# SmartBFT-Go/consensus

Hardware: NVIDIA H100
Metric: ECDSA-P256 verifies/sec at batch=64K (higher is better)
Workload: dtype u32 limbs (integer)

## Files before the change

consensus_b200/csrc/engine.cu:

```cuda
#include <cuda_runtime.h>
#include <dlfcn.h>

#include <algorithm>
#include <cstdarg>
#include <cstdio>
#include <cstdlib>
#include <cstring>
#include <mutex>
#include <string>
#include <vector>

#include "engine.h"
#include "sha256.cuh"
#include "quorum.cuh"

using namespace sbv;

namespace {

int env_int(const char *name, int dflt) {
    const char *v = getenv(name);
    return v && *v ? atoi(v) : dflt;
}

size_t fbytes(uint8_t curve) { return curve == SBV_P256 ? 32 : 48; }

bool is_pinned(const void *p) {
    cudaPointerAttributes a;
    if (cudaPointerGetAttributes(&a, p) != cudaSuccess) { cudaGetLastError(); return false; }
    return a.type == cudaMemoryTypeHost;
}

__global__ void k_mad_probe(uint32_t *out, uint32_t iters) {
    uint32_t a = threadIdx.x * 2654435761u + 12345u, b = blockIdx.x * 40503u + 777u;
    uint64_t acc[8];
#pragma unroll
    for (int i = 0; i < 8; i++) acc[i] = a + i;
    for (uint32_t it = 0; it < iters; it++) {
#pragma unroll
        for (int i = 0; i < 8; i++) acc[i] = (uint64_t)a * (uint32_t)(b + i) + acc[i];
        a ^= (uint32_t)acc[3];
    }
    uint64_t s = 0;
#pragma unroll
    for (int i = 0; i < 8; i++) s += acc[i];
    if (s == 0x1234567) out[0] = (uint32_t)s;
}

}

int sbv_ensure_scratch(sbv_engine *e, Dev &d, size_t bytes) {
    if (bytes <= d.scratch_cap) return 0;
    CU(e, cudaSetDevice(d.ordinal));
    if (d.d_scratch) cudaFree(d.d_scratch);
    d.d_scratch = nullptr;
    d.scratch_cap = 0;
    size_t cap = bytes + bytes / 4 + 4096;
    CU(e, cudaMalloc(&d.d_scratch, cap));
    d.scratch_cap = cap;
    return 0;
}

int sbv_lane_acquire(sbv_engine *e) {
    std::unique_lock<std::mutex> lk(e->mu);
    int lane = -1;
    e->lane_cv.wait(lk, [&] {
        for (int i = 0; i < SBV_LANES; i++)
            if (!e->lane_busy[i]) { lane = i; return true; }
        return false;
    });
    e->lane_busy[lane] = true;
    return lane;
}
void sbv_lane_release(sbv_engine *e, int lane) {
    { std::lock_guard<std::mutex> lk(e->mu); e->lane_busy[lane] = false; }
    e->lane_cv.notify_one();
}
int sbv_lane_ensure(sbv_engine *e, Dev &d, Dev::Lane &ln, size_t n, size_t pinned_bytes) {
    if (!ln.stream) CU(e, cudaStreamCreateWithFlags(&ln.stream, cudaStreamNonBlocking));
    if (n > ln.cap) {
        CU(e, cudaStreamSynchronize(ln.stream));
        uint8_t **ptrs[] = {&ln.d_r, &ln.d_s, &ln.d_qx, &ln.d_qy, &ln.d_dig, &ln.d_ok};
        for (auto p : ptrs) { if (*p) cudaFree(*p); *p = nullptr; }
        if (ln.d_slot) cudaFree(ln.d_slot);
        ln.d_slot = nullptr;
        ln.cap = 0;
        const size_t cap = n + n / 8 + 1024;
        CU(e, cudaMalloc(&ln.d_r, cap * 48));
        CU(e, cudaMalloc(&ln.d_s, cap * 48));
        CU(e, cudaMalloc(&ln.d_qx, cap * 48));
        CU(e, cudaMalloc(&ln.d_qy, cap * 48));
        CU(e, cudaMalloc(&ln.d_dig, cap * 64));
        CU(e, cudaMalloc(&ln.d_ok, cap));
        CU(e, cudaMalloc(&ln.d_slot, cap * 4));
        ln.cap = cap;
    }
    if (pinned_bytes > ln.h_pin_cap) {
        CU(e, cudaStreamSynchronize(ln.stream));
        if (ln.h_pin) cudaFreeHost(ln.h_pin);
        ln.h_pin = nullptr;
        ln.h_pin_cap = 0;
        const size_t cap = pinned_bytes + pinned_bytes / 4 + 4096;
        CU(e, cudaHostAlloc(&ln.h_pin, cap, cudaHostAllocPortable));
        ln.h_pin_cap = cap;
    }
    (void)d;
    return 0;
}
int sbv_lane_ensure_msgs(sbv_engine *e, Dev::Lane &ln, size_t bytes, size_t n_off) {
    if (!ln.stream) CU(e, cudaStreamCreateWithFlags(&ln.stream, cudaStreamNonBlocking));
    if (bytes > ln.msg_cap) {
        CU(e, cudaStreamSynchronize(ln.stream));
        if (ln.d_msgs) cudaFree(ln.d_msgs);
        ln.d_msgs = nullptr;
        ln.msg_cap = 0;
        const size_t cap = bytes + bytes / 8 + 4096;
        CU(e, cudaMalloc(&ln.d_msgs, cap));
        ln.msg_cap = cap;
    }
    if (n_off > ln.off_cap) {
        CU(e, cudaStreamSynchronize(ln.stream));
        if (ln.d_off) cudaFree(ln.d_off);
        if (ln.d_perm) cudaFree(ln.d_perm);
        ln.d_off = nullptr;
        ln.d_perm = nullptr;
        ln.off_cap = 0;
        const size_t cap = n_off + n_off / 8 + 1024;
        CU(e, cudaMalloc(&ln.d_off, cap * sizeof(uint64_t)));
        CU(e, cudaMalloc(&ln.d_perm, (cap + 3 * 1024) * sizeof(uint32_t)));
        ln.off_cap = cap;
    }
    return 0;
}
int sbv_lane_ensure_aux(sbv_engine *e, Dev::Lane &ln, size_t bytes) {
    if (!ln.stream) CU(e, cudaStreamCreateWithFlags(&ln.stream, cudaStreamNonBlocking));
    if (bytes <= ln.aux_cap) return 0;
    CU(e, cudaStreamSynchronize(ln.stream));
    if (ln.d_aux) cudaFree(ln.d_aux);
    if (ln.h_aux) cudaFreeHost(ln.h_aux);
    ln.d_aux = nullptr; ln.h_aux = nullptr; ln.aux_cap = 0;
    const size_t cap = bytes + bytes / 4 + 4096;
    CU(e, cudaMalloc(&ln.d_aux, cap));
    CU(e, cudaHostAlloc(&ln.h_aux, cap, cudaHostAllocPortable));
    ln.aux_cap = cap;
    return 0;
}
int sbv_launch_sha256(sbv_engine *e, size_t n, const uint8_t *d_msgs, const uint64_t *d_off, uint64_t base, uint8_t *d_digest, uint32_t *d_perm,
                      cudaStream_t st) {
    const uint32_t *perm = nullptr;
    if (d_perm && n >= 2048) {
        uint32_t *hist = d_perm + n, *start = hist + SHA_BINS, *cursor = start + SHA_BINS;
        CU(e, cudaMemsetAsync(hist, 0, SHA_BINS * sizeof(uint32_t), st));
        k_sha_hist<<<(uint32_t)((n + 255) / 256), 256, 0, st>>>((uint32_t)n, d_off, hist);
        k_sha_scan<<<1, SHA_BINS, 0, st>>>(hist, start, cursor);
        k_sha_scatter<<<(uint32_t)((n + 255) / 256), 256, 0, st>>>((uint32_t)n, d_off, start, cursor, d_perm);
        e->launches += 3;
        perm = d_perm;
    }
    k_sha256<<<(uint32_t)((n + 127) / 128), 128, 0, st>>>((uint32_t)n, d_msgs, d_off, base, d_digest, perm);
    e->launches += 1;
    CU(e, cudaGetLastError());
    return 0;
}
int sbv_lane_h2d(sbv_engine *e, Dev::Lane &ln, void *dst, const void *src, size_t bytes, size_t &stage_off, cudaStream_t st) {
    if (bytes == 0) return 0;
    if (!st) st = ln.stream;
    if (is_pinned(src)) {
        CU(e, cudaMemcpyAsync(dst, src, bytes, cudaMemcpyHostToDevice, st));
    } else {
        if (stage_off + bytes > ln.h_pin_cap) return fail(e, SBV_ERR_NOMEM, "pinned staging area too small (%zu + %zu > %zu)", stage_off, bytes, ln.h_pin_cap);
        memcpy(ln.h_pin + stage_off, src, bytes);
        CU(e, cudaMemcpyAsync(dst, ln.h_pin + stage_off, bytes, cudaMemcpyHostToDevice, st));
        stage_off += (bytes + 255) & ~(size_t)255;
    }
    return 0;
}

namespace {

struct NcclUniqueId { char internal[128]; };
typedef int (*nccl_comm_init_all_t)(void **comms, int ndev, const int *devlist);
typedef int (*nccl_comm_init_rank_t)(void **comm, int nranks, NcclUniqueId id, int rank);
typedef int (*nccl_get_unique_id_t)(NcclUniqueId *id);
typedef int (*nccl_comm_destroy_t)(void *comm);
typedef int (*nccl_group_t)(void);
typedef int (*nccl_all_gather_t)(const void *send, void *recv, size_t count, int dtype, void *comm, cudaStream_t st);
typedef const char *(*nccl_err_t)(int);
struct NcclApi {
    void *lib = nullptr;
    nccl_comm_init_all_t comm_init_all = nullptr;
    nccl_comm_init_rank_t comm_init_rank = nullptr;
    nccl_get_unique_id_t get_unique_id = nullptr;
    nccl_comm_destroy_t comm_destroy = nullptr;
    nccl_group_t group_start = nullptr, group_end = nullptr;
    nccl_all_gather_t all_gather = nullptr;
    nccl_err_t err_string = nullptr;
} g_nccl;
std::mutex g_nccl_mu;
constexpr int NCCL_UINT32 = 3;

int nccl_load(sbv_engine *e) {
    std::lock_guard<std::mutex> lk(g_nccl_mu);
    if (g_nccl.lib) return 0;
    void *h = dlopen("libnccl.so.2", RTLD_NOW | RTLD_LOCAL);
    if (!h) h = dlopen("libnccl.so", RTLD_NOW | RTLD_LOCAL);
    if (!h) return fail(e, SBV_ERR_NCCL, "cannot dlopen libnccl.so.2: %s", dlerror());
    g_nccl.comm_init_all = (nccl_comm_init_all_t)dlsym(h, "ncclCommInitAll");
    g_nccl.comm_init_rank = (nccl_comm_init_rank_t)dlsym(h, "ncclCommInitRank");
    g_nccl.get_unique_id = (nccl_get_unique_id_t)dlsym(h, "ncclGetUniqueId");
    g_nccl.comm_destroy = (nccl_comm_destroy_t)dlsym(h, "ncclCommDestroy");
    g_nccl.group_start = (nccl_group_t)dlsym(h, "ncclGroupStart");
    g_nccl.group_end = (nccl_group_t)dlsym(h, "ncclGroupEnd");
    g_nccl.all_gather = (nccl_all_gather_t)dlsym(h, "ncclAllGather");
    g_nccl.err_string = (nccl_err_t)dlsym(h, "ncclGetErrorString");
    if (!g_nccl.comm_init_all || !g_nccl.comm_init_rank || !g_nccl.get_unique_id || !g_nccl.comm_destroy || !g_nccl.group_start ||
        !g_nccl.group_end || !g_nccl.all_gather)
        return fail(e, SBV_ERR_NCCL, "libnccl lacks a required symbol");
    g_nccl.lib = h;
    return 0;
}
#define NC(e, call)                                                                                       \
    do {                                                                                                  \
        int _r = (call);                                                                                  \
        if (_r != 0)                                                                                      \
            return fail(e, SBV_ERR_NCCL, "%s failed: %s", #call, g_nccl.err_string ? g_nccl.err_string(_r) : "?"); \
    } while (0)

struct Shard { size_t lo, n; };
Shard shard_of(size_t n, int g, int G) {
    size_t lo = n * g / G, hi = n * (g + 1) / G;
    return {lo, hi - lo};
}

size_t words_per_shard(size_t n, int G) { return (((n + G - 1) / G) + 31) / 32; }

int gather_verdicts(sbv_engine *e, size_t n, int lane, size_t extra_words) {
    const int G = (int)e->devs.size();
    const size_t wp = words_per_shard(n, G) + extra_words;
    for (int g = 0; g < G; g++) {
        Dev &d = e->devs[g];
        CU(e, cudaSetDevice(d.ordinal));
        Dev::Lane &ln = d.lanes[lane];
        int rc = sbv_lane_ensure_aux(e, ln, wp * G * 4);
        if (rc) return rc;
    }
    for (int g = 0; g < G; g++) {
        Dev &d = e->devs[g];
        CU(e, cudaSetDevice(d.ordinal));
        Shard sh = shard_of(n, g, G);
        Dev::Lane &ln = d.lanes[lane];
        uint32_t *mine = (uint32_t *)ln.d_aux + wp * g;
        CU(e, cudaMemsetAsync(mine, 0, (wp - extra_words) * 4, ln.stream));
        if (sh.n) {
            k_pack_bits<<<(uint32_t)((sh.n + 255) / 256), 256, 0, ln.stream>>>((uint32_t)sh.n, ln.d_ok, mine);
            e->launches += 1;
            CU(e, cudaGetLastError());
        }
    }
    {
        std::lock_guard<std::mutex> lk(e->mu);
        NC(e, g_nccl.group_start());
        for (int g = 0; g < G; g++) {
            Dev &d = e->devs[g];
            uint32_t *buf = (uint32_t *)d.lanes[lane].d_aux;
            NC(e, g_nccl.all_gather(buf + wp * g, buf, wp, NCCL_UINT32, e->nccl_comms[g], d.lanes[lane].stream));
        }
        NC(e, g_nccl.group_end());
    }
    Dev &d0 = e->devs[0];
    CU(e, cudaSetDevice(d0.ordinal));
    CU(e, cudaMemcpyAsync(d0.lanes[lane].h_aux, d0.lanes[lane].d_aux, wp * G * 4, cudaMemcpyDeviceToHost, d0.lanes[lane].stream));
    return 0;
}

void unpack_verdicts(sbv_engine *e, size_t n, int lane, size_t extra_words, uint8_t *ok_host) {
    const int G = (int)e->devs.size();
    const size_t wp = words_per_shard(n, G) + extra_words;
    const uint32_t *words = (const uint32_t *)e->devs[0].lanes[lane].h_aux;
    for (int g = 0; g < G; g++) {
        Shard sh = shard_of(n, g, G);
        const uint32_t *w = words + wp * g;
        for (size_t i = 0; i < sh.n; i++) ok_host[sh.lo + i] = (w[i >> 5] >> (i & 31)) & 1u;
    }
}

int sync_lane(sbv_engine *e, int lane) {
    for (Dev &d : e->devs) {
        if (!d.lanes[lane].stream) continue;
        CU(e, cudaSetDevice(d.ordinal));
        CU(e, cudaStreamSynchronize(d.lanes[lane].stream));
    }
    return 0;
}

struct BatchSrc {
    const uint8_t *r, *s, *qx, *qy;
    const uint8_t *digest;
    uint8_t digest_len;
    const uint8_t *msgs;
    const uint64_t *msg_off;
};

int stage_and_verify(sbv_engine *e, Dev &d, int lane, uint8_t curve, size_t lo, size_t cnt, const BatchSrc &b, size_t extra_pinned = 0,
                     size_t *so_out = nullptr) {
    const size_t L = fbytes(curve);
    const bool hashing = b.digest == nullptr;
    const uint32_t dlen = hashing ? 32u : b.digest_len;
    Dev::Lane &ln = d.lanes[lane];
    CU(e, cudaSetDevice(d.ordinal));
    const uint64_t base = hashing ? b.msg_off[lo] : 0, bytes = hashing ? b.msg_off[lo + cnt] - base : 0;
    int chunks = 1;
    if (e->chunk_items > 0 && cnt >= (size_t)e->chunk_items) {
        chunks = (int)std::min<size_t>(std::max<size_t>(cnt / (size_t)e->chunk_items, 2), SBV_MAX_CHUNKS);
    }
    const size_t per = (((cnt + chunks - 1) / chunks) + 255) & ~(size_t)255;
    int rc = sbv_lane_ensure(e, d, ln, cnt ? cnt : 1, cnt * (4 * L + dlen + 1) + bytes + (cnt + 1) * 8 + (size_t)(4 * chunks + 8) * 256 + extra_pinned);
    if (rc) return rc;
    if (hashing && (rc = sbv_lane_ensure_msgs(e, ln, bytes + 16, cnt + 1))) return rc;
    cudaStream_t up = ln.stream;
    if (chunks > 1) {
        if (!ln.stream2) {
            CU(e, cudaStreamCreateWithFlags(&ln.stream2, cudaStreamNonBlocking));
            CU(e, cudaEventCreateWithFlags(&ln.ev_a, cudaEventDisableTiming));
            CU(e, cudaEventCreateWithFlags(&ln.ev_b, cudaEventDisableTiming));
        }
        for (int c = 0; c < chunks; c++)
            if (!ln.ev_chunk[c]) CU(e, cudaEventCreateWithFlags(&ln.ev_chunk[c], cudaEventDisableTiming));
        up = ln.stream2;
    }
    size_t so = 0;
    if ((rc = sbv_lane_h2d(e, ln, ln.d_qx, b.qx + lo * L, cnt * L, so))) return rc;
    if ((rc = sbv_lane_h2d(e, ln, ln.d_qy, b.qy + lo * L, cnt * L, so))) return rc;
    VerifyLaunch vl;
    {
        std::lock_guard<std::mutex> lk(e->mu);
        if ((rc = sbv_launch_verify_begin(e, d, curve, cnt, ln.d_qx, ln.d_qy, ln.stream, &vl, chunks))) return rc;
    }
    auto abandon = [&](int code) {
        std::lock_guard<std::mutex> lk(e->mu);
        sbv_launch_verify_abort(vl, ln.stream);
        return code;
    };
    for (int c = 0; c < chunks; c++) {
        const size_t clo = (size_t)c * per < cnt ? (size_t)c * per : cnt, cn = cnt - clo < per ? cnt - clo : per;
        const size_t g = lo + clo;
        if (hashing && cn) {
            const uint64_t o = b.msg_off[g] - base, len = b.msg_off[g + cn] - b.msg_off[g];
            rc = sbv_lane_h2d(e, ln, ln.d_msgs + o, b.msgs + b.msg_off[g], len, so, up);
            if (!rc) rc = sbv_lane_h2d(e, ln, ln.d_off + clo, b.msg_off + g, (cn + 1) * 8, so, up);
        } else if (cn) {
            rc = sbv_lane_h2d(e, ln, ln.d_dig + clo * dlen, b.digest + g * dlen, cn * dlen, so, up);
        }
        if (!rc) rc = sbv_lane_h2d(e, ln, ln.d_r + clo * L, b.r + g * L, cn * L, so, up);
        if (!rc) rc = sbv_lane_h2d(e, ln, ln.d_s + clo * L, b.s + g * L, cn * L, so, up);
        if (rc) return abandon(rc);
        if (chunks > 1) {
            cudaError_t ce = cudaEventRecord(ln.ev_chunk[c], up);
            if (ce == cudaSuccess) ce = cudaStreamWaitEvent(ln.stream, ln.ev_chunk[c], 0);
            if (ce != cudaSuccess) return abandon(sbv_fail(e, SBV_ERR_CUDA, "chunk event: %s", cudaGetErrorString(ce)));
        }
        if (hashing && cn && (rc = sbv_launch_sha256(e, cn, ln.d_msgs, ln.d_off + clo, base, ln.d_dig + clo * 32, ln.d_perm + clo, ln.stream)))
            return abandon(rc);
        std::lock_guard<std::mutex> lk(e->mu);
        if (chunks == 1) rc = sbv_launch_verify_finish(e, d, vl, ln.d_r, ln.d_s, ln.d_dig, dlen, ln.d_ok, ln.stream);
        else rc = sbv_launch_verify_chunk(e, d, vl, c, clo, cn, c == chunks - 1, ln.d_r, ln.d_s, ln.d_dig, dlen, ln.d_ok, ln.stream);
        if (rc) { sbv_launch_verify_abort(vl, ln.stream); return rc; }
    }
    if (so_out) *so_out = so;
    return 0;
}

}

extern "C" {

int sbv_create(const int *device_ordinals, int n_devices, sbv_engine **out) {
    if (!out || n_devices < 1 || n_devices > 8) return SBV_ERR_ARG;
    *out = nullptr;
    int count = 0;
    if (cudaGetDeviceCount(&count) != cudaSuccess || count < n_devices) return SBV_ERR_CUDA;
    sbv_engine *e = new sbv_engine();
    e->keyed_warp_limit = env_int("SBV_KEYED_WARP_LIMIT", 2048);
    e->group_threshold = env_int("SBV_GROUP_THRESHOLD", 16);
    e->group_max_keys = env_int("SBV_GROUP_MAX_KEYS", 8192);
    e->group_min_batch = env_int("SBV_GROUP_MIN_BATCH", 0);
    e->gsplit = env_int("SBV_GSPLIT", 1) != 0;
    e->chunk_items = env_int("SBV_CHUNK_ITEMS", 262144);
    e->gather_hi = env_int("SBV_GATHER_PRIORITY", 1) != 0;
    e->tab_hi = env_int("SBV_TAB_PRIORITY", 1) != 0;
    {
        uint64_t t = (uint64_t)(uintptr_t)e;
        FILE *f = fopen("/dev/urandom", "rb");
        if (f) { if (fread(&t, sizeof t, 1, f) != 1) t ^= 0x9e3779b97f4a7c15ull; fclose(f); }
        e->hash_seed = (uint32_t)(t ^ (t >> 32)) | 1u;
    }
    e->devs.resize(n_devices);
    for (int g = 0; g < n_devices; g++) {
        Dev &d = e->devs[g];
        d.ordinal = device_ordinals ? device_ordinals[g] : g;
        cudaError_t st = cudaSetDevice(d.ordinal);
        if (st == cudaSuccess) st = cudaStreamCreateWithFlags(&d.stream, cudaStreamNonBlocking);
        if (st == cudaSuccess && sbv_init_gtables(e, d) != 0) st = cudaErrorUnknown;
        if (st != cudaSuccess) {
            fprintf(stderr, "sbv_create: device %d: %s (%s)\n", d.ordinal, cudaGetErrorString(st), e->err.c_str());
            sbv_destroy(e);
            return SBV_ERR_CUDA;
        }
    }
    if (n_devices > 1) {
        std::vector<int> ords;
        for (Dev &d : e->devs) ords.push_back(d.ordinal);
        e->nccl_comms.assign(n_devices, nullptr);
        if (nccl_load(e) != 0 || g_nccl.comm_init_all(e->nccl_comms.data(), n_devices, ords.data()) != 0) {
            fprintf(stderr, "sbv_create: NCCL initialisation failed: %s\n", e->err.c_str());
            e->nccl_comms.clear();
            sbv_destroy(e);
            return SBV_ERR_NCCL;
        }
    }
    *out = e;
    return SBV_OK;
}

void sbv_destroy(sbv_engine *e) {
    if (!e) return;
    for (Dev &d : e->devs) {
        cudaSetDevice(d.ordinal);
        cudaDeviceSynchronize();
    }
    for (void *c : e->nccl_comms) if (c && g_nccl.comm_destroy) g_nccl.comm_destroy(c);
    for (void *c : e->rank_comms) if (c && g_nccl.comm_destroy) g_nccl.comm_destroy(c);
    for (auto &hi : e->rank_hi) {
        if (hi.st) cudaStreamDestroy(hi.st);
        if (hi.in) cudaEventDestroy(hi.in);
        if (hi.out) cudaEventDestroy(hi.out);
    }
    for (Dev &d : e->devs) {
        cudaSetDevice(d.ordinal);
        void *ptrs[] = {d.gtab[0], d.gtab[1], d.d_scratch};
        for (void *p : ptrs) if (p) cudaFree(p);
        sbv_scratch_free(d);
        sbv_keys_free(d);
        for (auto &ln : d.lanes) {
            void *lp[] = {ln.d_r, ln.d_s, ln.d_qx, ln.d_qy, ln.d_dig, ln.d_ok, ln.d_slot, ln.d_msgs, ln.d_off, ln.d_perm, ln.d_aux};
            for (void *p : lp) if (p) cudaFree(p);
            if (ln.h_pin) cudaFreeHost(ln.h_pin);
            if (ln.h_aux) cudaFreeHost(ln.h_aux);
            if (ln.stream) cudaStreamDestroy(ln.stream);
            if (ln.stream2) cudaStreamDestroy(ln.stream2);
            if (ln.ev_a) cudaEventDestroy(ln.ev_a);
            if (ln.ev_b) cudaEventDestroy(ln.ev_b);
        }
        for (cudaEvent_t ev : d.prof_events) cudaEventDestroy(ev);
        if (d.stream) cudaStreamDestroy(d.stream);
    }
    delete e;
}

const char *sbv_last_error(const sbv_engine *e) {
    static thread_local std::string copy;
    if (!e) return "null engine";
    sbv_engine *m = const_cast<sbv_engine *>(e);
    std::lock_guard<std::mutex> lk(m->err_mu);
    copy = m->err;
    return copy.c_str();
}
int sbv_device_count(const sbv_engine *e) { return e ? (int)e->devs.size() : 0; }
uint64_t sbv_kernel_launches(const sbv_engine *e) { return e ? e->launches.load() : 0; }

void sbv_compute_quorum(uint64_t n, uint32_t *q, uint32_t *f) {
    uint64_t ff = n ? (n - 1) / 3 : 0;
    if (f) *f = (uint32_t)ff;
    if (q) *q = (uint32_t)((n + ff + 2) / 2);
}

int sbv_verify_batch_device(sbv_engine *e, int device_index, uint8_t curve, size_t n, const uint8_t *d_r,
                            const uint8_t *d_s, const uint8_t *d_qx, const uint8_t *d_qy, const uint8_t *d_digest,
                            uint8_t digest_len, uint8_t *d_ok, void *cuda_stream) {
    if (!e || curve > SBV_P384 || device_index < 0 || device_index >= (int)e->devs.size() || digest_len == 0)
        return fail(e, SBV_ERR_ARG, "sbv_verify_batch_device: bad argument");
    if (n == 0) return SBV_OK;
    if (n > 0x7fffffffu || (digest_len & 3) || digest_len > 64) return fail(e, SBV_ERR_ARG, "n too large or digest_len not a multiple of 4");
    if (!d_r || !d_s || !d_qx || !d_qy || !d_digest || !d_ok) return fail(e, SBV_ERR_ARG, "null buffer");
    std::lock_guard<std::mutex> lk(e->mu);
    Dev &d = e->devs[device_index];
    CU(e, cudaSetDevice(d.ordinal));
    cudaStream_t st = (cudaStream_t)cuda_stream;
    return sbv_launch_verify(e, d, curve, n, d_r, d_s, d_qx, d_qy, d_digest, digest_len, d_ok, st);
}

int sbv_verify_batch(sbv_engine *e, uint8_t curve, size_t n, const uint8_t *r, const uint8_t *s, const uint8_t *qx,
                     const uint8_t *qy, const uint8_t *digest, uint8_t digest_len, uint8_t *ok) {
    if (!e || curve > SBV_P384 || digest_len == 0 || (digest_len & 3) || digest_len > 64)
        return fail(e, SBV_ERR_ARG, "sbv_verify_batch: bad argument");
    if (n == 0) return SBV_OK;
    if (!r || !s || !qx || !qy || !digest || !ok) return fail(e, SBV_ERR_ARG, "null buffer");
    if (n > 0x7fffffffu) return fail(e, SBV_ERR_ARG, "n too large");
    const int G = (int)e->devs.size();
    LaneGuard guard(e);
    const int lane = guard.lane;
    if (G == 1) {
        Dev &d = e->devs[0];
        int rc = stage_and_verify(e, d, lane, curve, 0, n, BatchSrc{r, s, qx, qy, digest, digest_len, nullptr, nullptr});
        if (rc) return rc;
        CU(e, cudaMemcpyAsync(ok, d.lanes[lane].d_ok, n, cudaMemcpyDeviceToHost, d.lanes[lane].stream));
        return sync_lane(e, lane);
    }
    for (int g = 0; g < G; g++) {
        Shard sh = shard_of(n, g, G);
        if (sh.n == 0) continue;
        int rc = stage_and_verify(e, e->devs[g], lane, curve, sh.lo, sh.n, BatchSrc{r, s, qx, qy, digest, digest_len, nullptr, nullptr});
        if (rc) return rc;
    }
    int rc = gather_verdicts(e, n, lane, 0);
    if (rc) return rc;
    if ((rc = sync_lane(e, lane))) return rc;
    unpack_verdicts(e, n, lane, 0, ok);
    return SBV_OK;
}

int sbv_comm_unique_id(uint8_t *id128) {
    if (!id128) return SBV_ERR_ARG;
    if (nccl_load(nullptr) != 0) return SBV_ERR_NCCL;
    NcclUniqueId id;
    if (g_nccl.get_unique_id(&id) != 0) return SBV_ERR_NCCL;
    memcpy(id128, id.internal, 128);
    return SBV_OK;
}

int sbv_comm_init_rank(sbv_engine *e, const uint8_t *id128, int nranks, int rank) {
    if (!e || !id128 || nranks < 1 || rank < 0 || rank >= nranks || e->devs.size() != 1)
        return fail(e, SBV_ERR_ARG, "sbv_comm_init_rank: bad argument (needs a single-device engine)");
    if (!e->rank_comms.empty() && (e->nranks != nranks || e->rank != rank)) return fail(e, SBV_ERR_ARG, "sbv_comm_init_rank: rank / nranks changed");
    if (int rc = nccl_load(e)) return rc;
    Dev &d = e->devs[0];
    CU(e, cudaSetDevice(d.ordinal));
    NcclUniqueId id;
    memcpy(id.internal, id128, 128);
    void *comm = nullptr;
    NC(e, g_nccl.comm_init_rank(&comm, nranks, id, rank));
    sbv_engine::ChannelHi hi;
    if (e->gather_hi) {
        int lo_p = 0, hi_p = 0;
        CU(e, cudaDeviceGetStreamPriorityRange(&lo_p, &hi_p));
        CU(e, cudaStreamCreateWithPriority(&hi.st, cudaStreamNonBlocking, hi_p));
        CU(e, cudaEventCreateWithFlags(&hi.in, cudaEventDisableTiming));
        CU(e, cudaEventCreateWithFlags(&hi.out, cudaEventDisableTiming));
    }
    std::lock_guard<std::mutex> lk(e->mu);
    e->rank_comms.push_back(comm);
    e->rank_hi.push_back(hi);
    e->rank = rank;
    e->nranks = nranks;
    return (int)e->rank_comms.size() - 1;
}

int sbv_comm_ranks(const sbv_engine *e) { return e ? e->nranks : 0; }

int sbv_gather_verdicts_device(sbv_engine *e, int channel, const uint8_t *d_ok, size_t n, uint32_t *d_mask_all, void *cuda_stream) {
    if (!e || e->devs.size() != 1 || !d_ok || !d_mask_all || n == 0 || n > 0x7fffffffu) return fail(e, SBV_ERR_ARG, "sbv_gather_verdicts_device: bad argument");
    Dev &d = e->devs[0];
    CU(e, cudaSetDevice(d.ordinal));
    cudaStream_t st = (cudaStream_t)cuda_stream;
    const size_t wp = (n + 31) / 32;
    uint32_t *mine = d_mask_all + wp * (size_t)e->rank;
    if (e->nranks > 1 && (channel < 0 || channel >= (int)e->rank_comms.size())) return fail(e, SBV_ERR_NCCL, "no such channel: call sbv_comm_init_rank first");
    const bool fork = e->nranks > 1 && e->rank_hi[channel].st;
    cudaStream_t gs = st;
    if (fork) {
        const sbv_engine::ChannelHi &hi = e->rank_hi[channel];
        CU(e, cudaEventRecord(hi.in, st));
        CU(e, cudaStreamWaitEvent(hi.st, hi.in, 0));
        gs = hi.st;
    }
    k_pack_bits<<<(uint32_t)((n + 255) / 256), 256, 0, gs>>>((uint32_t)n, d_ok, mine);
    e->launches += 1;
    CU(e, cudaGetLastError());
    if (e->nranks > 1) NC(e, g_nccl.all_gather(mine, d_mask_all, wp, NCCL_UINT32, e->rank_comms[channel], gs));
    if (fork) {
        const sbv_engine::ChannelHi &hi = e->rank_hi[channel];
        CU(e, cudaEventRecord(hi.out, gs));
        CU(e, cudaStreamWaitEvent(st, hi.out, 0));
    }
    return SBV_OK;
}

int sbv_gather_words_device(sbv_engine *e, int channel, uint32_t *d_all, size_t words, void *cuda_stream) {
    if (!e || e->devs.size() != 1 || !d_all || words == 0) return fail(e, SBV_ERR_ARG, "sbv_gather_words_device: bad argument");
    if (e->nranks == 1) return SBV_OK;
    if (channel < 0 || channel >= (int)e->rank_comms.size()) return fail(e, SBV_ERR_NCCL, "no such channel: call sbv_comm_init_rank first");
    CU(e, cudaSetDevice(e->devs[0].ordinal));
    NC(e, g_nccl.all_gather(d_all + words * (size_t)e->rank, d_all, words, NCCL_UINT32, e->rank_comms[channel], (cudaStream_t)cuda_stream));
    return SBV_OK;
}

int sbv_verify_batch_ranked(sbv_engine *e, int channel, uint8_t curve, size_t n, const uint8_t *r, const uint8_t *s, const uint8_t *qx,
                            const uint8_t *qy, const uint8_t *digest, uint8_t digest_len, uint8_t *ok, uint32_t *mask_all) {
    if (!e || curve > SBV_P384 || digest_len == 0 || (digest_len & 3) || digest_len > 64 || e->devs.size() != 1)
        return fail(e, SBV_ERR_ARG, "sbv_verify_batch_ranked: bad argument");
    if (n == 0 || n > 0x7fffffffu) return fail(e, SBV_ERR_ARG, "n must be in [1, 2^31)");
    if (!r || !s || !qx || !qy || !digest || !ok || !mask_all) return fail(e, SBV_ERR_ARG, "null buffer");
    LaneGuard guard(e);
    const int lane = guard.lane;
    Dev &d = e->devs[0];
    Dev::Lane &ln = d.lanes[lane];
    int rc = stage_and_verify(e, d, lane, curve, 0, n, BatchSrc{r, s, qx, qy, digest, digest_len, nullptr, nullptr});
    if (rc) return rc;
    const size_t wp = (n + 31) / 32;
    if ((rc = sbv_lane_ensure_aux(e, ln, wp * (size_t)e->nranks * 4))) return rc;
    CU(e, cudaMemcpyAsync(ok, ln.d_ok, n, cudaMemcpyDeviceToHost, ln.stream));
    if ((rc = sbv_gather_verdicts_device(e, channel, ln.d_ok, n, (uint32_t *)ln.d_aux, ln.stream))) return rc;
    CU(e, cudaMemcpyAsync(mask_all, ln.d_aux, wp * (size_t)e->nranks * 4, cudaMemcpyDeviceToHost, ln.stream));
    return sync_lane(e, lane);
}

void *sbv_host_alloc(size_t bytes) {
    void *p = nullptr;
    if (cudaHostAlloc(&p, bytes ? bytes : 1, cudaHostAllocPortable) != cudaSuccess) { cudaGetLastError(); return nullptr; }
    return p;
}
void sbv_host_free(void *p) { if (p) cudaFreeHost(p); }

double sbv_probe_mad_rate(sbv_engine *e) {
    if (!e) return 0.0;
    std::lock_guard<std::mutex> lk(e->mu);
    Dev &d = e->devs[0];
    if (cudaSetDevice(d.ordinal) != cudaSuccess) return 0.0;
    if (sbv_ensure_scratch(e, d, 4096)) return 0.0;
    cudaDeviceProp prop;
    cudaGetDeviceProperties(&prop, d.ordinal);
    const uint32_t iters = 4096;
    const int blocks = prop.multiProcessorCount * 8, threads = 256;
    cudaEvent_t a, b;
    cudaEventCreate(&a);
    cudaEventCreate(&b);
    k_mad_probe<<<blocks, threads, 0, d.stream>>>((uint32_t *)d.d_scratch, 64);
    float best = 1e30f;
    for (int rep = 0; rep < 5; rep++) {
        cudaEventRecord(a, d.stream);
        k_mad_probe<<<blocks, threads, 0, d.stream>>>((uint32_t *)d.d_scratch, iters);
        cudaEventRecord(b, d.stream);
        if (cudaStreamSynchronize(d.stream) != cudaSuccess) return 0.0;
        float ms = 0;
        cudaEventElapsedTime(&ms, a, b);
        if (ms < best) best = ms;
    }
    e->launches += 6;
    cudaEventDestroy(a);
    cudaEventDestroy(b);
    double macs = (double)blocks * threads * (double)iters * 8.0;
    return macs / (best * 1e-3);
}

}

#include "engine_more.inc"

extern "C" {

int sbv_profile_enable(sbv_engine *e, int on) {
    if (!e) return SBV_ERR_ARG;
    std::lock_guard<std::mutex> lk(e->mu);
    e->profiling = on != 0;
    for (Dev &d : e->devs) d.prof_used = 0;
    return SBV_OK;
}

int sbv_profile_read(sbv_engine *e, double *prep_ms, double *verify_ms, uint64_t *n_launches) {
    if (!e) return SBV_ERR_ARG;
    std::lock_guard<std::mutex> lk(e->mu);
    double p = 0, v = 0;
    uint64_t cnt = 0;
    for (Dev &d : e->devs) {
        CU(e, cudaSetDevice(d.ordinal));
        for (size_t i = 0; i + 4 < d.prof_used && i + 4 < d.prof_events.size(); i += 5) {
            float a = 0, b = 0, g = 0;
            CU(e, cudaEventSynchronize(d.prof_events[i + 3]));
            CU(e, cudaEventElapsedTime(&a, d.prof_events[i], d.prof_events[i + 1]));
            CU(e, cudaEventElapsedTime(&b, d.prof_events[i + 2], d.prof_events[i + 3]));
            CU(e, cudaEventElapsedTime(&g, d.prof_events[i + 1], d.prof_events[i + 4]));
            p += a; v += b + g; cnt++;
        }
        d.prof_used = 0;
    }
    if (prep_ms) *prep_ms = p;
    if (verify_ms) *verify_ms = v;
    if (n_launches) *n_launches = cnt;
    return SBV_OK;
}

}
```

consensus_b200/csrc/engine.h:

```cpp
#pragma once
#include <cuda_runtime.h>

#include <atomic>
#include <cstdarg>
#include <cstdio>
#include <cstdint>
#include <condition_variable>
#include <mutex>
#include <string>
#include <vector>

#include "../../include/sbv.h"
#include "ops.h"

constexpr int SBV_LANES = 6;
constexpr int SBV_SCRATCH = 8;
constexpr int SBV_MAX_CHUNKS = 32;

struct Dev {
    int ordinal = 0;
    cudaStream_t stream = nullptr;
    uint32_t *gtab[2] = {nullptr, nullptr};
    struct Scratch {
        size_t cap = 0;
        size_t kcap = 0;
        uint32_t *uw = nullptr;
        uint8_t *flags = nullptr;
        uint32_t *tscr = nullptr;
        uint32_t *gacc = nullptr;
        uint32_t hsize = 0;
        uint32_t *htab = nullptr, *rep = nullptr, *keylist = nullptr, *klist = nullptr, *glist = nullptr;
        uint32_t *zeroed = nullptr;
        int32_t *keyid = nullptr, *item_kid = nullptr;
        uint32_t *bases = nullptr, *hs = nullptr, *ztop = nullptr, *pref = nullptr, *ktab = nullptr;
        uint8_t *keyflags = nullptr;
        cudaStream_t s_tab = nullptr, s_gen = nullptr;
        cudaEvent_t done = nullptr, ev_group = nullptr, ev_prep = nullptr, ev_tab = nullptr, ev_gen = nullptr;
        bool used = false;
        bool open = false;
        struct Caps {
            size_t uw = 0, flags = 0, tscr = 0, gacc = 0, htab = 0, rep = 0, keylist = 0, klist = 0, glist = 0, zeroed = 0, keyid = 0, item_kid = 0, bases = 0,
                   hs = 0, ztop = 0, pref = 0, ktab = 0, keyflags = 0;
        } caps;
    } ws[SBV_SCRATCH];
    unsigned ws_next = 0;
    struct Lane {
        cudaStream_t stream = nullptr;
        size_t cap = 0;
        uint8_t *d_r = nullptr, *d_s = nullptr, *d_qx = nullptr, *d_qy = nullptr, *d_dig = nullptr, *d_ok = nullptr;
        uint32_t *d_slot = nullptr;
        uint8_t *d_msgs = nullptr;
        uint64_t *d_off = nullptr;
        uint32_t *d_perm = nullptr;
        size_t msg_cap = 0, off_cap = 0;
        uint8_t *h_pin = nullptr;
        size_t h_pin_cap = 0;
        uint8_t *d_aux = nullptr, *h_aux = nullptr;
        size_t aux_cap = 0;
        cudaStream_t stream2 = nullptr;
        cudaEvent_t ev_a = nullptr, ev_b = nullptr;
        cudaEvent_t ev_chunk[SBV_MAX_CHUNKS] = {};
    } lanes[SBV_LANES];
    uint8_t *d_scratch = nullptr;
    size_t scratch_cap = 0;
    uint32_t *ktab[2] = {nullptr, nullptr};
    uint8_t *keyflags[2] = {nullptr, nullptr};
    int32_t *slot2local[2] = {nullptr, nullptr};
    uint32_t n_slots = 0, n_local[2] = {0, 0};
    std::vector<cudaEvent_t> prof_events;
    size_t prof_used = 0;
};

struct sbv_engine {
    std::vector<Dev> devs;
    std::mutex mu;
    std::mutex err_mu;
    std::condition_variable lane_cv;
    bool lane_busy[SBV_LANES] = {};
    std::string err;
    std::atomic<uint64_t> launches{0};
    int keyed_warp_limit = 2048;
    int group_threshold = 16;
    int group_max_keys = 8192;
    int group_min_batch = 0;
    int chunk_items = 262144;
    bool gsplit = true;
    uint32_t hash_seed = 0x9e3779b9u;
    bool profiling = false;
    void *nccl_lib = nullptr;
    std::vector<void *> nccl_comms;
    std::vector<void *> rank_comms;
    struct ChannelHi { cudaStream_t st = nullptr; cudaEvent_t in = nullptr, out = nullptr; };
    std::vector<ChannelHi> rank_hi;
    bool gather_hi = true;
    bool tab_hi = true;
    int rank = 0, nranks = 1;
    uint64_t verification_seq = 0;
    std::vector<uint64_t> key_ids;
    std::vector<uint8_t> key_curve;
    std::vector<uint8_t> key_xy;
};

inline int sbv_fail(sbv_engine *e, int code, const char *fmt, ...) {
    char buf[512];
    va_list ap;
    va_start(ap, fmt);
    vsnprintf(buf, sizeof buf, fmt, ap);
    va_end(ap);
    if (e) {
        std::lock_guard<std::mutex> lk(e->err_mu);
        e->err = buf;
    }
    return code;
}
#define fail sbv_fail

#define CU(e, call)                                                                                   \
    do {                                                                                              \
        cudaError_t _st = (call);                                                                     \
        if (_st != cudaSuccess)                                                                       \
            return sbv_fail(e, SBV_ERR_CUDA, "%s failed: %s (%s:%d)", #call, cudaGetErrorString(_st), \
                            __FILE__, __LINE__);                                                      \
    } while (0)

struct VerifyLaunch {
    Dev::Scratch *w = nullptr;
    cudaEvent_t *ev = nullptr;
    const uint8_t *d_qx = nullptr, *d_qy = nullptr;
    size_t n = 0;
    uint8_t curve = 0;
    bool grouping = false;
    int chunks = 1;
};

int sbv_launch_verify(sbv_engine *e, Dev &d, uint8_t curve, size_t n, const uint8_t *d_r, const uint8_t *d_s, const uint8_t *d_qx,
                      const uint8_t *d_qy, const uint8_t *d_dig, uint32_t dlen, uint8_t *d_ok, cudaStream_t st);
int sbv_launch_verify_begin(sbv_engine *e, Dev &d, uint8_t curve, size_t n, const uint8_t *d_qx, const uint8_t *d_qy, cudaStream_t st, VerifyLaunch *vl,
                            int chunks = 1);
void sbv_launch_verify_abort(const VerifyLaunch &vl, cudaStream_t st);
int sbv_launch_verify_chunk(sbv_engine *e, Dev &d, const VerifyLaunch &vl, int c, size_t lo, size_t cn, bool last, const uint8_t *d_r, const uint8_t *d_s,
                            const uint8_t *d_dig, uint32_t dlen, uint8_t *d_ok, cudaStream_t st);
int sbv_launch_verify_finish(sbv_engine *e, Dev &d, const VerifyLaunch &vl, const uint8_t *d_r, const uint8_t *d_s, const uint8_t *d_dig, uint32_t dlen,
                             uint8_t *d_ok, cudaStream_t st);
int sbv_launch_keyed(sbv_engine *e, Dev &d, uint8_t curve, size_t n, const uint32_t *d_slot, const uint8_t *d_r, const uint8_t *d_s,
                     const uint8_t *d_dig, uint32_t dlen, uint8_t *d_ok, cudaStream_t st);
int sbv_init_gtables(sbv_engine *e, Dev &d);
int sbv_keys_build(sbv_engine *e, Dev &d);
void sbv_keys_free(Dev &d);
void sbv_scratch_free(Dev &d);

int sbv_lane_acquire(sbv_engine *e);
void sbv_lane_release(sbv_engine *e, int lane);
int sbv_lane_ensure(sbv_engine *e, Dev &d, Dev::Lane &ln, size_t n, size_t pinned_bytes);
int sbv_lane_ensure_msgs(sbv_engine *e, Dev::Lane &ln, size_t bytes, size_t n_off);
int sbv_lane_ensure_aux(sbv_engine *e, Dev::Lane &ln, size_t bytes);
int sbv_launch_sha256(sbv_engine *e, size_t n, const uint8_t *d_msgs, const uint64_t *d_off, uint64_t base, uint8_t *d_digest, uint32_t *d_perm,
                      cudaStream_t st);
int sbv_lane_h2d(sbv_engine *e, Dev::Lane &ln, void *dst, const void *src, size_t bytes, size_t &stage_off, cudaStream_t st = nullptr);
int sbv_ensure_scratch(sbv_engine *e, Dev &d, size_t bytes);

struct LaneGuard {
    sbv_engine *e;
    int lane;
    explicit LaneGuard(sbv_engine *eng) : e(eng), lane(sbv_lane_acquire(eng)) {}
    ~LaneGuard() {
        for (Dev &d : e->devs) {
            if (!d.lanes[lane].stream) continue;
            cudaSetDevice(d.ordinal);
            if (d.lanes[lane].stream2) cudaStreamSynchronize(d.lanes[lane].stream2);
            cudaStreamSynchronize(d.lanes[lane].stream);
        }
        sbv_lane_release(e, lane);
    }
    LaneGuard(const LaneGuard &) = delete;
    LaneGuard &operator=(const LaneGuard &) = delete;
};
```

consensus_b200/csrc/inst_common.cuh:

```cuda
#pragma once
#include "keygroup.cuh"
#include "ops.h"
#include <cstdlib>

namespace sbv {

template <class C> struct Cfg;
template <> struct Cfg<P256> { static constexpr int COZ_MINB = 6, KT_MINB = 7, KT_VARIANT = 2, COMB_MINB = 6; static constexpr bool COMB_INL = true; };
template <> struct Cfg<P384> { static constexpr int COZ_MINB = 4, KT_MINB = 4, KT_VARIANT = 0; };

template <class C>
cudaError_t op_gtable_init(uint32_t *gtab, cudaStream_t st) {
    const size_t entries = (size_t)C::GWINS << C::GW;
    k_gtable_init<C><<<(unsigned)((entries + 127) / 128), 128, 0, st>>>(gtab);
    return cudaGetLastError();
}

template <class C>
cudaError_t op_prep(uint32_t n, const uint8_t *r, const uint8_t *s, const uint8_t *dig, uint32_t dlen, uint32_t *uw, uint8_t *flags,
                    cudaStream_t st) {
    return launch_prep<C, 8>(n, r, s, dig, dlen, uw, flags, st);
}

template <class C>
cudaError_t op_group(uint32_t n, const uint8_t *qx, const uint8_t *qy, uint32_t seed, uint32_t hmask, uint32_t *htab, uint32_t *rep,
                     uint32_t *kcnt, uint32_t threshold, uint32_t max_keys, int32_t *keyid, uint32_t *keylist, int32_t *item_kid,
                     uint32_t *klist, uint32_t *glist, uint32_t *counters, int route, cudaStream_t st) {
    const unsigned blocks = (n + 255) / 256;
    k_kg_insert<C><<<blocks, 256, 0, st>>>(n, qx, qy, seed, hmask, htab, rep, kcnt);
    k_kg_assign<<<blocks, 256, 0, st>>>(n, rep, kcnt, threshold, max_keys, keyid, keylist, counters);
    if (route) k_kg_route<<<blocks, 256, 0, st>>>(n, rep, keyid, item_kid, klist, glist, counters);
    return cudaGetLastError();
}

[[maybe_unused]] static cudaError_t op_route(uint32_t n, const uint32_t *rep, const int32_t *keyid, int32_t *item_kid, uint32_t *klist, uint32_t *glist,
                            uint32_t *counters, cudaStream_t st) {
    k_kg_route<<<(n + 255) / 256, 256, 0, st>>>(n, rep, keyid, item_kid, klist, glist, counters);
    return cudaGetLastError();
}

template <class C>
cudaError_t op_gpart(uint32_t n, const uint32_t *uw, const uint32_t *gtab, uint32_t *gacc, cudaStream_t st) {
    constexpr int BLOCK = 64;
    k_gpart<C, BLOCK, Cfg<C>::KT_MINB - 1><<<(n + BLOCK - 1) / BLOCK, BLOCK, 0, st>>>(n, uw, reinterpret_cast<const uint4 *>(gtab), gacc);
    return cudaGetLastError();
}

template <class C>
cudaError_t op_coz(uint32_t n, const uint8_t *qx, const uint8_t *qy, const uint8_t *r, const uint32_t *uw, const uint8_t *flags,
                   const uint32_t *gtab, uint32_t *tscr, uint8_t *ok, const uint32_t *list, const uint32_t *count, cudaStream_t st) {
    constexpr int BLOCK = 64;
    const size_t smem = (size_t)7 * 2 * C::N * 4 * BLOCK;
    k_verify_coz<C, BLOCK, Cfg<C>::COZ_MINB><<<(n + BLOCK - 1) / BLOCK, BLOCK, smem, st>>>(
        n, qx, qy, r, uw, flags, reinterpret_cast<const uint4 *>(gtab), tscr, ok, list, count);
    return cudaGetLastError();
}

template <class C, int W>
cudaError_t op_kt_build(const uint32_t *nkeys_ptr, uint32_t cap, const uint32_t *keylist, const uint8_t *qx, const uint8_t *qy,
                        uint32_t *bases, uint32_t *hs, uint32_t *ztop, uint32_t *pref, uint32_t *ktab, uint8_t *keyflags, cudaStream_t st) {
    using KT = KeyTab<32 * C::N, W>;
    const unsigned kb = (cap + 63) / 64;
    const unsigned wb = (unsigned)(((size_t)cap * KT::NWIN + 63) / 64);
    static const int bases_variant = getenv("SBV_KT_BASES") ? atoi(getenv("SBV_KT_BASES")) : 0;
    if (bases_variant == 2) k_kt_bases<C, KT, false><<<kb, 64, 0, st>>>(nkeys_ptr, cap, keylist, qx, qy, bases, keyflags);
    else if (bases_variant == 1) k_kt_bases<C, KT, true><<<kb, 64, 0, st>>>(nkeys_ptr, cap, keylist, qx, qy, bases, keyflags);
    else k_kt_bases4<C, KT><<<(unsigned)(((size_t)cap * 4 + 127) / 128), 128, 0, st>>>(nkeys_ptr, cap, keylist, qx, qy, bases, keyflags);
    k_kt_fill<C, W><<<wb, 64, 0, st>>>(nkeys_ptr, cap, bases, keyflags, hs, ztop, ktab);
    k_kt_inv<C, KT><<<kb, 64, 0, st>>>(nkeys_ptr, cap, keyflags, ztop, pref);
    k_kt_final<C, KT><<<wb, 64, 0, st>>>(nkeys_ptr, cap, bases, keyflags, hs, ztop, ktab);
    return cudaGetLastError();
}

template <class C, int W>
cudaError_t op_kt_verify(int reg, int warp, uint32_t n, const uint32_t *slot, const int32_t *kidmap, uint32_t n_slots,
                         const uint8_t *keyflags, const uint8_t *r, const uint32_t *uw, const uint8_t *flags, const uint32_t *gtab,
                         const uint32_t *ktab, uint8_t *ok, const uint32_t *list, const uint32_t *count, const uint32_t *gacc, cudaStream_t st) {
    constexpr int BLOCK = 64, MINB = Cfg<C>::KT_MINB;
    static const int variant = getenv("SBV_KT_VARIANT") ? atoi(getenv("SBV_KT_VARIANT")) : Cfg<C>::KT_VARIANT;
    const uint4 *g4 = reinterpret_cast<const uint4 *>(gtab), *k4 = reinterpret_cast<const uint4 *>(ktab);
    const unsigned blocks = (n + BLOCK - 1) / BLOCK;
#define SBV_KT_ARGS n, slot, kidmap, n_slots, keyflags, r, uw, flags, g4, k4, ok, list, count, gacc
    if (warp) {
        k_verify_kt_warp<C, W><<<(unsigned)(((size_t)n * 32 + 127) / 128), 128, 0, st>>>(n, slot, kidmap, n_slots, keyflags, r, uw, flags, g4, k4, ok);
    } else if (reg) {
        if (variant == 1) k_verify_kt<C, W, BLOCK, MINB, true, true><<<blocks, BLOCK, 0, st>>>(SBV_KT_ARGS);
        else if (variant == 2) k_verify_kt<C, W, BLOCK, MINB - 1, true, true><<<blocks, BLOCK, 0, st>>>(SBV_KT_ARGS);
        else k_verify_kt<C, W, BLOCK, MINB, true, false><<<blocks, BLOCK, 0, st>>>(SBV_KT_ARGS);
    } else {
        if (variant == 1) k_verify_kt<C, W, BLOCK, MINB, false, true><<<blocks, BLOCK, 0, st>>>(SBV_KT_ARGS);
        else if (variant == 2) k_verify_kt<C, W, BLOCK, MINB - 1, false, true><<<blocks, BLOCK, 0, st>>>(SBV_KT_ARGS);
        else k_verify_kt<C, W, BLOCK, MINB, false, false><<<blocks, BLOCK, 0, st>>>(SBV_KT_ARGS);
    }
#undef SBV_KT_ARGS
    return cudaGetLastError();
}

template <class C>
cudaError_t op_comb_build(const uint32_t *nkeys_ptr, uint32_t cap, const uint32_t *keylist, const uint8_t *qx, const uint8_t *qy,
                          uint32_t *bases, uint32_t *hs, uint32_t *ztop, uint32_t *pref, uint32_t *ktab, uint8_t *keyflags, cudaStream_t st) {
    using CT = CombTab<C>;
    const unsigned kb = (cap + 63) / 64;
    const unsigned cb = (unsigned)(((size_t)cap * CT::NCHAIN + 63) / 64);
    k_kt_bases4<C, CT><<<(unsigned)(((size_t)cap * 4 + 127) / 128), 128, 0, st>>>(nkeys_ptr, cap, keylist, qx, qy, bases, keyflags);
    k_comb_affine<C><<<kb, 64, 0, st>>>(nkeys_ptr, cap, keyflags, bases, pref);
    k_comb_fill<C><<<cb, 64, 0, st>>>(nkeys_ptr, cap, bases, keyflags, hs, ztop, ktab);
    k_kt_inv<C, CT><<<kb, 64, 0, st>>>(nkeys_ptr, cap, keyflags, ztop, pref);
    k_kt_final<C, CT><<<cb, 64, 0, st>>>(nkeys_ptr, cap, bases, keyflags, hs, ztop, ktab);
    return cudaGetLastError();
}

template <class C>
cudaError_t op_comb_verify(int reg, int warp, uint32_t n, const uint32_t *slot, const int32_t *kidmap, uint32_t n_slots,
                           const uint8_t *keyflags, const uint8_t *r, const uint32_t *uw, const uint8_t *flags, const uint32_t *gtab,
                           const uint32_t *ktab, uint8_t *ok, const uint32_t *list, const uint32_t *count, const uint32_t *gacc, cudaStream_t st) {
    constexpr int BLOCK = 64;
    (void)slot; (void)n_slots;
    if (reg || warp || !list || !count) return cudaErrorInvalidValue;
    k_verify_comb<C, BLOCK, Cfg<C>::COMB_MINB, Cfg<C>::COMB_INL><<<(n + BLOCK - 1) / BLOCK, BLOCK, 0, st>>>(
        n, kidmap, keyflags, r, uw, flags, reinterpret_cast<const uint4 *>(gtab), reinterpret_cast<const uint4 *>(ktab), ok, list, count, gacc);
    return cudaGetLastError();
}

template <class C, class KT>
constexpr KtGeom kt_geom() {
    using KS = KtSizes<C, KT>;
    return KtGeom{KS::bases_words(1), KS::hs_words(1), KS::ztop_words(1), KS::ktab_words(1)};
}

}
```

consensus_b200/csrc/inst_p256_comb.cu:

```cuda
#include "inst_common.cuh"
using namespace sbv;
const KtOps sbv_comb_p256 = {kt_geom<P256, CombTab<P256>>(), op_comb_build<P256>, op_comb_verify<P256>};
```

consensus_b200/csrc/kernels.cuh:

```cuda
#pragma once
#include "curve.cuh"

namespace sbv {

template <int BITS, int W>
struct Windows {
    static constexpr int COUNT = (BITS + 1 + W - 1) / W;
    static constexpr int ENTRIES = 1 << (W - 1);
};

template <class C>
SBV_DEV void load_affine(uint32_t (&x)[C::N], uint32_t (&y)[C::N], const uint4 *src) {
    constexpr int N = C::N;
#pragma unroll
    for (int i = 0; i < N / 4; i++) {
        uint4 v = __ldg(src + i);
        x[4 * i] = v.x; x[4 * i + 1] = v.y; x[4 * i + 2] = v.z; x[4 * i + 3] = v.w;
        uint4 u = __ldg(src + N / 4 + i);
        y[4 * i] = u.x; y[4 * i + 1] = u.y; y[4 * i + 2] = u.z; y[4 * i + 3] = u.w;
    }
}

template <class C>
__global__ void k_gtable_init(uint32_t *__restrict__ gtab) {
    constexpr int N = C::N;
    const int t = blockIdx.x * blockDim.x + threadIdx.x;
    if (t >= C::GWINS << C::GW) return;
    const int win = t >> C::GW, b = t & ((1 << C::GW) - 1);
    uint32_t *out = gtab + (size_t)t * 2 * N;
    if (b == 0) {
        for (int i = 0; i < 2 * N; i++) out[i] = 0;
        return;
    }
    Jac<C> base;
    C::get_gx(base.X); C::get_gy(base.Y); C::get_one(base.Z);
    for (int i = 0; i < C::GW * win; i++) pt_double<C>(base);
    Jac<C> acc;
    C::get_one(acc.X); C::get_one(acc.Y);
#pragma unroll
    for (int i = 0; i < N; i++) acc.Z[i] = 0;
    for (int bit = C::GW - 1; bit >= 0; bit--) {
        pt_double<C>(acc);
        pt_add<C, false>(acc, base.X, base.Y, base.Z, false, !((b >> bit) & 1));
    }
    uint32_t zi[N], zi2[N], zi3[N], x[N], y[N];
    f_inv<C>(zi, acc.Z);
    C::fsqr(zi2, zi);
    C::fmul(zi3, zi2, zi);
    C::fmul(x, acc.X, zi2);
    C::fmul(y, acc.Y, zi3);
    for (int i = 0; i < N; i++) { out[i] = x[i]; out[N + i] = y[i]; }
}

template <class C>
SBV_DEV void load_digest(uint32_t (&e)[C::N], const uint8_t *d, uint32_t dlen) {
    constexpr int N = C::N;
    if (dlen == (uint32_t)C::BYTES) { load_be<N>(e, d); return; }
    const int L = dlen < (uint32_t)C::BYTES ? (int)dlen : C::BYTES;
#pragma unroll
    for (int j = 0; j < N; j++) {
        uint32_t v = 0;
#pragma unroll
        for (int k = 0; k < 4; k++) {
            int pos = L - 1 - (4 * j + k);
            uint32_t byte = pos >= 0 ? (uint32_t)d[pos] : 0u;
            v |= byte << (8 * k);
        }
        e[j] = v;
    }
}

template <class C>
SBV_DEV uint32_t comb_digit_u1(const uint32_t *__restrict__ uw, uint32_t n, uint32_t idx, int win) {
    const int pos = win * C::GW;
    return (__ldg(uw + (size_t)(pos >> 5) * n + idx) >> (pos & 31)) & ((1u << C::GW) - 1u);
}
template <class C, int W>
SBV_DEV int booth_digit_u2(const uint32_t *__restrict__ uw, uint32_t n, uint32_t idx, int win) {
    constexpr int N = C::N;
    const uint32_t *u2 = uw + (size_t)N * n + idx;
    const int pos = W * win - 1;
    uint32_t b;
    if (pos < 0) {
        b = (__ldg(u2) << 1) & ((2u << W) - 1);
    } else {
        const int wd = pos >> 5, sh = pos & 31;
        const uint32_t lo = wd < N ? __ldg(u2 + (size_t)wd * n) : 0u;
        const uint32_t hi = wd + 1 < N ? __ldg(u2 + (size_t)(wd + 1) * n) : 0u;
        b = __funnelshift_r(lo, hi, sh) & ((2u << W) - 1);
    }
    const uint32_t sign = b >> W;
    uint32_t d = sign ? (((2u << W) - 1) - b) : b;
    d = (d + 1) >> 1;
    return sign ? -(int)d : (int)d;
}

template <class C, int S>
__global__ void __launch_bounds__(128) k_prep(uint32_t n, const uint8_t *__restrict__ r_be, const uint8_t *__restrict__ s_be,
                                              const uint8_t *__restrict__ dig_be, uint32_t dlen,
                                              uint32_t *__restrict__ uw, uint8_t *__restrict__ flags) {
    constexpr int N = C::N;
    const uint32_t T = gridDim.x * blockDim.x;
    const uint32_t t = blockIdx.x * blockDim.x + threadIdx.x;
    uint32_t sm[S][N];
    uint32_t pref[S][N];
    uint32_t nmod[N], rr[N];
    C::get_n(nmod);
    C::get_rr_n(rr);
    uint32_t run[N];
    C::get_one_n(run);
    int cnt = 0;
#pragma unroll 1
    for (int k = 0; k < S; k++) {
        uint32_t idx = t + (uint32_t)k * T;
        if (idx >= n) break;
        uint32_t s[N], r[N];
        load_be<N>(s, s_be + (size_t)idx * C::BYTES);
        load_be<N>(r, r_be + (size_t)idx * C::BYTES);
        bool ok = !mp_is_zero<N>(s) && mp_lt<N>(s, nmod) && !mp_is_zero<N>(r) && mp_lt<N>(r, nmod);
        flags[idx] = ok ? 1 : 0;
        uint32_t one[N];
#pragma unroll
        for (int i = 0; i < N; i++) one[i] = (i == 0);
        uint32_t sv[N];
        mp_select<N>(sv, ok, s, one);
        uint32_t m[N];
        C::nmul(m, sv, rr);
        C::nmul(run, run, m);
#pragma unroll
        for (int i = 0; i < N; i++) { sm[k][i] = m[i]; pref[k][i] = run[i]; }
        cnt++;
    }
    if (cnt == 0) return;
    uint32_t inv[N];
    n_inv<C>(inv, run);
#pragma unroll 1
    for (int k = cnt - 1; k >= 0; k--) {
        uint32_t idx = t + (uint32_t)k * T;
        uint32_t w[N], m[N];
#pragma unroll
        for (int i = 0; i < N; i++) m[i] = sm[k][i];
        if (k > 0) {
            uint32_t pv[N];
#pragma unroll
            for (int i = 0; i < N; i++) pv[i] = pref[k - 1][i];
            C::nmul(w, inv, pv);
            C::nmul(inv, inv, m);
        } else {
            mp_copy<N>(w, inv);
        }
        uint32_t e[N], r[N], u1[N], u2[N];
        load_digest<C>(e, dig_be + (size_t)idx * dlen, dlen);
        load_be<N>(r, r_be + (size_t)idx * C::BYTES);
        C::nmul(u1, e, w);
        C::nmul(u2, r, w);
#pragma unroll
        for (int i = 0; i < N; i++) {
            uw[(size_t)i * n + idx] = u1[i];
            uw[(size_t)(N + i) * n + idx] = u2[i];
        }
    }
}

#ifdef __CUDACC__
template <class C, int S>
inline cudaError_t launch_prep(uint32_t n, const uint8_t *d_r, const uint8_t *d_s, const uint8_t *d_dig, uint32_t dlen, uint32_t *uw,
                               uint8_t *flags, cudaStream_t st) {
    constexpr int PB = 128;
    const uint32_t pthreads = (n + S - 1) / S;
    k_prep<C, S><<<(pthreads + PB - 1) / PB, PB, 0, st>>>(n, d_r, d_s, d_dig, dlen, uw, flags);
    return cudaGetLastError();
}
#endif

template <class C>
SBV_DEV bool final_check(const Jac<C> &acc, const uint8_t *__restrict__ r_be, uint32_t idx) {
    constexpr int N = C::N;
    bool match = false;
    if (!mp_is_zero<N>(acc.Z)) {
        uint32_t zz[N], r[N], rr[N], rm[N], lhs[N], pmn[N];
        C::fsqr(zz, acc.Z);
        load_be<N>(r, r_be + (size_t)idx * C::BYTES);
        C::get_rr_p(rr);
        C::fmul(rm, r, rr);
        C::fmul(lhs, rm, zz);
        match = mp_eq<N>(lhs, acc.X);
        C::get_p_minus_n(pmn);
        if (!match && mp_lt<N>(r, pmn)) {
            uint32_t r2[N], nmod[N];
            C::get_n(nmod);
            mp_add<N>(r2, r, nmod);
            C::fmul(rm, r2, rr);
            C::fmul(lhs, rm, zz);
            match = mp_eq<N>(lhs, acc.X);
        }
    }
    return match;
}

template <class C>
SBV_DEV bool load_key(uint32_t (&qxm)[C::N], uint32_t (&qym)[C::N], const uint8_t *__restrict__ qx_be, const uint8_t *__restrict__ qy_be, uint32_t idx) {
    constexpr int N = C::N;
    uint32_t x[N], y[N], rr[N], pmod[N];
    C::get_p(pmod);
    load_be<N>(x, qx_be + (size_t)idx * C::BYTES);
    load_be<N>(y, qy_be + (size_t)idx * C::BYTES);
    bool good = mp_lt<N>(x, pmod) && mp_lt<N>(y, pmod);
    C::get_rr_p(rr);
    C::fmul(qxm, x, rr);
    C::fmul(qym, y, rr);
    uint32_t lhs[N], rhs[N], t[N], b[N];
    C::fsqr(lhs, qym);
    C::fsqr(t, qxm);
    C::fmul(rhs, t, qxm);
    C::fsub(rhs, rhs, qxm); C::fsub(rhs, rhs, qxm); C::fsub(rhs, rhs, qxm);
    C::get_b(b);
    C::fadd(rhs, rhs, b);
    return good && mp_eq<N>(lhs, rhs);
}

template <class C>
SBV_DEV void add_u1G(Jac<C> &acc, const uint32_t *__restrict__ uw, uint32_t n, uint32_t idx, const uint4 *__restrict__ gtab) {
    constexpr int N = C::N;
    constexpr int EU4 = 2 * N / 4;
    uint32_t one[N];
    C::get_one(one);
    uint32_t gx[N], gy[N];
    uint32_t gb = comb_digit_u1<C>(uw, n, idx, 0);
    load_affine<C>(gx, gy, gtab + (size_t)gb * EU4);
#pragma unroll 1
    for (int win = 0; win < C::GWINS; win++) {
        uint32_t ngx[N], ngy[N];
        uint32_t ngb = 0;
        if (win + 1 < C::GWINS) {
            ngb = comb_digit_u1<C>(uw, n, idx, win + 1);
            load_affine<C>(ngx, ngy, gtab + (((size_t)(win + 1) << C::GW) + ngb) * EU4);
        }
        pt_add<C, true>(acc, gx, gy, one, false, gb == 0);
        if (win + 1 < C::GWINS) { mp_copy<N>(gx, ngx); mp_copy<N>(gy, ngy); gb = ngb; }
    }
}

template <class C, int BLOCK, int MINB>
__global__ void __launch_bounds__(BLOCK, MINB) k_verify_coz(uint32_t n, const uint8_t *__restrict__ qx_be, const uint8_t *__restrict__ qy_be,
                                                             const uint8_t *__restrict__ r_be, const uint32_t *__restrict__ uw,
                                                             const uint8_t *__restrict__ flags,
                                                             const uint4 *__restrict__ gtab, uint32_t *__restrict__ tscr,
                                                             uint8_t *__restrict__ ok_out, const uint32_t *__restrict__ list,
                                                             const uint32_t *__restrict__ count) {
    constexpr int N = C::N;
    constexpr int W = 4;
    constexpr int NWIN = Windows<32 * N, W>::COUNT;
    extern __shared__ uint32_t tab[];
    const uint32_t tid = threadIdx.x;
    const uint32_t t = blockIdx.x * BLOCK + tid;
    if (t >= (list ? __ldg(count) : n)) return;
    const uint32_t idx = list ? __ldg(list + t) : t;
#define TAB(k, c, w) tab[((((k) - 2) * 2 + (c)) * N + (w)) * BLOCK + tid]
#define SCR(w) tscr[(size_t)(w) * n + t]
    uint32_t one[N];
    C::get_one(one);
    {
        uint32_t qxm[N], qym[N];
        const bool good = load_key<C>(qxm, qym, qx_be, qy_be, idx) && flags[idx] != 0;
        if (!good) { ok_out[idx] = 0; return; }
        Jac<C> P;
        mp_copy<N>(P.X, qxm); mp_copy<N>(P.Y, qym); mp_copy<N>(P.Z, one);
        pt_double<C>(P);
#pragma unroll
        for (int i = 0; i < N; i++) { TAB(2, 0, i) = P.X[i]; TAB(2, 1, i) = P.Y[i]; SCR(5 * N + i) = P.Z[i]; }
#pragma unroll 1
        for (int k = 3; k <= 8; k++) {
            uint32_t h[N];
            pt_madd_table<C>(P, qxm, qym, h);
#pragma unroll
            for (int i = 0; i < N; i++) { TAB(k, 0, i) = P.X[i]; TAB(k, 1, i) = P.Y[i]; SCR((5 + k - 2) * N + i) = h[i]; }
        }
        {
            uint32_t z2[N], z3[N];
            C::fsqr(z2, P.Z);
            C::fmul(z3, z2, P.Z);
#pragma unroll
            for (int i = 0; i < N; i++) { SCR(2 * N + i) = P.Z[i]; SCR(3 * N + i) = z2[i]; SCR(4 * N + i) = z3[i]; }
        }
        uint32_t cacc[N];
        mp_copy<N>(cacc, one);
#pragma unroll 1
        for (int j = 7; j >= 1; j--) {
            uint32_t h[N], c2[N], c3[N], xx[N], yy[N];
#pragma unroll
            for (int i = 0; i < N; i++) h[i] = SCR((5 + j + 1 - 2) * N + i);
            C::fmul(cacc, cacc, h);
            C::fsqr(c2, cacc);
            C::fmul(c3, c2, cacc);
            if (j >= 2) {
#pragma unroll
                for (int i = 0; i < N; i++) { xx[i] = TAB(j, 0, i); yy[i] = TAB(j, 1, i); }
            } else {
                mp_copy<N>(xx, qxm); mp_copy<N>(yy, qym);
            }
            C::fmul(xx, xx, c2);
            C::fmul(yy, yy, c3);
            if (j >= 2) {
#pragma unroll
                for (int i = 0; i < N; i++) { TAB(j, 0, i) = xx[i]; TAB(j, 1, i) = yy[i]; }
            } else {
#pragma unroll
                for (int i = 0; i < N; i++) { SCR(i) = xx[i]; SCR(N + i) = yy[i]; }
            }
        }
    }
    Jac<C> acc;
    mp_copy<N>(acc.X, one);
    mp_copy<N>(acc.Y, one);
#pragma unroll
    for (int i = 0; i < N; i++) acc.Z[i] = 0;

#pragma unroll 1
    for (int win = NWIN - 1; win >= 0; win--) {
        if (win != NWIN - 1) {
#pragma unroll 1
            for (int k = 0; k < W; k++) pt_double<C>(acc);
        }
        const int d = booth_digit_u2<C, W>(uw, n, idx, win);
        bool neg = d < 0, skip = d == 0;
        int e = neg ? -d : d;
        int es = e < 2 ? 2 : e;
        uint32_t x2[N], y2[N], zc[N], zc2[N], zc3[N];
#pragma unroll
        for (int i = 0; i < N; i++) {
            uint32_t sx = TAB(es, 0, i), sy = TAB(es, 1, i);
            uint32_t gx1 = SCR(i), gy1 = SCR(N + i);
            x2[i] = e == 1 ? gx1 : sx;
            y2[i] = e == 1 ? gy1 : sy;
            zc[i] = SCR(2 * N + i); zc2[i] = SCR(3 * N + i); zc3[i] = SCR(4 * N + i);
        }
        pt_add_m<C, 2>(acc, x2, y2, zc, zc2, zc3, neg, skip);
    }
    add_u1G<C>(acc, uw, n, idx, gtab);
#undef TAB
#undef SCR
    ok_out[idx] = final_check<C>(acc, r_be, idx) ? 1 : 0;
}

template <int BITS, int W>
struct KeyTab {
    static constexpr int NWIN = Windows<BITS, W>::COUNT;
    static constexpr int ENT = Windows<BITS, W>::ENTRIES;
    static constexpr int NBASE = NWIN, STEP = W, NCHAIN = NWIN;
    static constexpr size_t POINTS = (size_t)NWIN * ENT;
};

template <class C>
struct CombTab {
    static constexpr int TEETH = 8, BLOCKS = 2, NBASE = TEETH * BLOCKS;
    static constexpr int SPACING = 32 * C::N / NBASE;
    static constexpr int STEP = SPACING;
    static constexpr int NCHAIN = BLOCKS * 16, ENT = 16;
    static constexpr size_t POINTS = (size_t)NCHAIN * ENT;
    static_assert(SPACING * NBASE == 32 * C::N, "the rows cover the scalar exactly");
    SBV_DEV static uint32_t slot(int b, uint32_t m) {
        const uint32_t g = m & 15u;
        return ((uint32_t)b * 16u + (m >> 4)) * 16u + (g ^ (g >> 1) ^ (g >> 2) ^ (g >> 3));
    }
};

template <class C>
SBV_DEV uint32_t comb_mask_u2(const uint32_t *__restrict__ uw, uint32_t n, uint32_t idx, int b, int j) {
    using CT = CombTab<C>;
    const uint32_t *u2 = uw + (size_t)C::N * n + idx;
    uint32_t m = 0;
#pragma unroll
    for (int t = 0; t < CT::TEETH; t++) {
        const int pos = CT::SPACING * (CT::TEETH * b + t) + j;
        m |= ((__ldg(u2 + (size_t)(pos >> 5) * n) >> (pos & 31)) & 1u) << t;
    }
    return m;
}

template <class C>
struct Inl : C {
    SBV_DEV static void fmul(uint32_t (&r)[C::N], const uint32_t (&a)[C::N], const uint32_t (&b)[C::N]) { C::fmul_inline(r, a, b); }
    SBV_DEV static void fsqr(uint32_t (&r)[C::N], const uint32_t (&a)[C::N]) { C::fsqr_inline(r, a); }
};
template <class C, bool INL> struct PickArith { using type = C; };
template <class C> struct PickArith<C, true> { using type = Inl<C>; };

template <class C, int BLOCK, int MINB>
__global__ void __launch_bounds__(BLOCK, MINB) k_gpart(uint32_t n, const uint32_t *__restrict__ uw, const uint4 *__restrict__ gtab,
                                                        uint32_t *__restrict__ gacc) {
    constexpr int N = C::N;
    const uint32_t idx = blockIdx.x * BLOCK + threadIdx.x;
    if (idx >= n) return;
    Jac<C> acc;
    C::get_one(acc.X);
    C::get_one(acc.Y);
#pragma unroll
    for (int i = 0; i < N; i++) acc.Z[i] = 0;
    add_u1G<C>(acc, uw, n, idx, gtab);
#pragma unroll
    for (int i = 0; i < N; i++) {
        gacc[(size_t)i * n + idx] = acc.X[i];
        gacc[(size_t)(N + i) * n + idx] = acc.Y[i];
        gacc[(size_t)(2 * N + i) * n + idx] = acc.Z[i];
    }
}

template <class C, int W, int BLOCK, int MINB, bool REG, bool INL>
__global__ void __launch_bounds__(BLOCK, MINB) k_verify_kt(uint32_t n, const uint32_t *__restrict__ slot, const int32_t *__restrict__ kidmap,
                                                            uint32_t n_slots, const uint8_t *__restrict__ keyflags,
                                                            const uint8_t *__restrict__ r_be, const uint32_t *__restrict__ uw,
                                                            const uint8_t *__restrict__ flags, const uint4 *__restrict__ gtab,
                                                            const uint4 *__restrict__ ktab, uint8_t *__restrict__ ok_out,
                                                            const uint32_t *__restrict__ list, const uint32_t *__restrict__ count,
                                                            const uint32_t *__restrict__ gacc) {
    using A = typename PickArith<C, INL>::type;
    constexpr int N = C::N;
    constexpr int EU4 = 2 * N / 4;
    using KT = KeyTab<32 * N, W>;
    const int TOTAL = gacc ? KT::NWIN : KT::NWIN + C::GWINS;
    const uint32_t t = blockIdx.x * BLOCK + threadIdx.x;
    if (t >= (list ? __ldg(count) : n)) return;
    const uint32_t idx = list ? __ldg(list + t) : t;
    bool good = flags[idx] != 0;
    int32_t kid;
    if (REG) {
        const uint32_t sl = slot[idx];
        kid = sl < n_slots ? kidmap[sl] : -1;
    } else {
        kid = kidmap[idx];
    }
    good = good && kid >= 0 && keyflags[kid < 0 ? 0 : kid] != 0;
    if (!good) { ok_out[idx] = 0; return; }
    const uint4 *kt = ktab + (size_t)kid * KT::POINTS * EU4;
    uint32_t one[N];
    C::get_one(one);
    Jac<A> acc;
    if (gacc) {
#pragma unroll
        for (int i = 0; i < N; i++) {
            acc.X[i] = __ldg(gacc + (size_t)i * n + idx);
            acc.Y[i] = __ldg(gacc + (size_t)(N + i) * n + idx);
            acc.Z[i] = __ldg(gacc + (size_t)(2 * N + i) * n + idx);
        }
    } else {
        mp_copy<N>(acc.X, one);
        mp_copy<N>(acc.Y, one);
#pragma unroll
        for (int i = 0; i < N; i++) acc.Z[i] = 0;
    }
    auto fetch = [&](int w, uint32_t (&x)[N], uint32_t (&y)[N], bool &neg, bool &skip) {
        if (w < KT::NWIN) {
            const int d = booth_digit_u2<C, W>(uw, n, idx, w);
            const int e = d < 0 ? -d : d;
            load_affine<C>(x, y, kt + ((size_t)w * KT::ENT + (e ? e - 1 : 0)) * EU4);
            neg = d < 0; skip = d == 0;
        } else {
            const int g = w - KT::NWIN;
            const uint32_t b = comb_digit_u1<C>(uw, n, idx, g);
            load_affine<C>(x, y, gtab + (((size_t)g << C::GW) + b) * EU4);
            neg = false; skip = b == 0;
        }
    };
    uint32_t cx[N], cy[N];
    bool cneg, cskip;
    fetch(0, cx, cy, cneg, cskip);
#pragma unroll 1
    for (int w = 0; w < TOTAL; w++) {
        uint32_t nx[N], ny[N];
        bool nneg = false, nskip = true;
        if (w + 1 < TOTAL) fetch(w + 1, nx, ny, nneg, nskip);
        pt_add<A, true>(acc, cx, cy, one, cneg, cskip);
        if (w + 1 < TOTAL) { mp_copy<N>(cx, nx); mp_copy<N>(cy, ny); cneg = nneg; cskip = nskip; }
    }
    Jac<C> fin;
    mp_copy<N>(fin.X, acc.X); mp_copy<N>(fin.Y, acc.Y); mp_copy<N>(fin.Z, acc.Z);
    ok_out[idx] = final_check<C>(fin, r_be, idx) ? 1 : 0;
}

template <class C, int BLOCK, int MINB, bool INL>
__global__ void __launch_bounds__(BLOCK, MINB) k_verify_comb(uint32_t n, const int32_t *__restrict__ kidmap, const uint8_t *__restrict__ keyflags,
                                                              const uint8_t *__restrict__ r_be, const uint32_t *__restrict__ uw,
                                                              const uint8_t *__restrict__ flags, const uint4 *__restrict__ gtab,
                                                              const uint4 *__restrict__ ktab, uint8_t *__restrict__ ok_out,
                                                              const uint32_t *__restrict__ list, const uint32_t *__restrict__ count,
                                                              const uint32_t *__restrict__ gacc) {
    using A = typename PickArith<C, INL>::type;
    constexpr int N = C::N;
    constexpr int EU4 = 2 * N / 4;
    using CT = CombTab<C>;
    constexpr int KADD = CT::SPACING * CT::BLOCKS;
    const int TOTAL = gacc ? KADD : KADD + C::GWINS;
    const uint32_t t = blockIdx.x * BLOCK + threadIdx.x;
    if (t >= __ldg(count)) return;
    const uint32_t idx = __ldg(list + t);
    const int32_t kid = kidmap[idx];
    const bool good = flags[idx] != 0 && kid >= 0 && keyflags[kid < 0 ? 0 : kid] != 0;
    if (!good) { ok_out[idx] = 0; return; }
    const uint4 *kt = ktab + (size_t)kid * CT::POINTS * EU4;
    uint32_t one[N];
    C::get_one(one);
    Jac<A> acc;
    mp_copy<N>(acc.X, one);
    mp_copy<N>(acc.Y, one);
#pragma unroll
    for (int i = 0; i < N; i++) acc.Z[i] = 0;
    auto fetch = [&](int s, uint32_t (&x)[N], uint32_t (&y)[N], bool &skip) {
        if (s < KADD) {
            const int b = s & 1;
            const uint32_t m = comb_mask_u2<C>(uw, n, idx, b, CT::SPACING - 1 - (s >> 1));
            load_affine<C>(x, y, kt + (size_t)CT::slot(b, m) * EU4);
            skip = m == 0;
        } else {
            const int g = s - KADD;
            const uint32_t d = comb_digit_u1<C>(uw, n, idx, g);
            load_affine<C>(x, y, gtab + (((size_t)g << C::GW) + d) * EU4);
            skip = d == 0;
        }
    };
    uint32_t cx[N], cy[N];
    bool cskip;
    fetch(0, cx, cy, cskip);
    int s = 0, dbl = 0;
#pragma unroll 1
    while (s < TOTAL || dbl) {
        if (dbl) {
            pt_double<A>(acc);
            dbl--;
            continue;
        }
        uint32_t nx[N], ny[N];
        bool nskip = true;
        if (s + 1 < TOTAL) fetch(s + 1, nx, ny, nskip);
        dbl = pt_add_m<A, 1, true>(acc, cx, cy, one, one, one, false, cskip) ? 1 : 0;
        s++;
        if (s < KADD && (s & 1) == 0) dbl++;
        if (s < TOTAL) { mp_copy<N>(cx, nx); mp_copy<N>(cy, ny); cskip = nskip; }
    }
    Jac<C> fin;
    mp_copy<N>(fin.X, acc.X); mp_copy<N>(fin.Y, acc.Y); mp_copy<N>(fin.Z, acc.Z);
    if (gacc) {
        Jac<C> g;
#pragma unroll
        for (int i = 0; i < N; i++) {
            g.X[i] = __ldg(gacc + (size_t)i * n + idx);
            g.Y[i] = __ldg(gacc + (size_t)(N + i) * n + idx);
            g.Z[i] = __ldg(gacc + (size_t)(2 * N + i) * n + idx);
        }
        pt_add<C, false>(fin, g.X, g.Y, g.Z, false, mp_is_zero<N>(g.Z));
    }
    ok_out[idx] = final_check<C>(fin, r_be, idx) ? 1 : 0;
}

template <class C, int W>
__global__ void __launch_bounds__(128) k_verify_kt_warp(uint32_t n, const uint32_t *__restrict__ slot, const int32_t *__restrict__ slot2local,
                                                        uint32_t n_slots, const uint8_t *__restrict__ keyflags,
                                                        const uint8_t *__restrict__ r_be, const uint32_t *__restrict__ uw,
                                                        const uint8_t *__restrict__ flags,
                                                        const uint4 *__restrict__ gtab, const uint4 *__restrict__ ktab,
                                                        uint8_t *__restrict__ ok_out) {
    constexpr int N = C::N;
    constexpr int EU4 = 2 * N / 4;
    using KT = KeyTab<32 * N, W>;
    const uint32_t idx = (blockIdx.x * blockDim.x + threadIdx.x) >> 5;
    const uint32_t lane = threadIdx.x & 31;
    if (idx >= n) return;
    bool good = flags[idx] != 0;
    const uint32_t sl = slot[idx];
    int32_t local = sl < n_slots ? slot2local[sl] : -1;
    good = good && local >= 0;
    if (local < 0) local = 0;
    good = good && keyflags[local] != 0;
    const uint4 *kt = ktab + (size_t)local * KT::POINTS * EU4;
    uint32_t one[N];
    C::get_one(one);
    Jac<C> acc;
    mp_copy<N>(acc.X, one);
    mp_copy<N>(acc.Y, one);
#pragma unroll
    for (int i = 0; i < N; i++) acc.Z[i] = 0;
#pragma unroll 1
    for (int it = 0; it < (KT::NWIN + 31) / 32; it++) {
        const int win = it * 32 + (int)lane;
        const bool live = win < KT::NWIN;
        const int d = live ? booth_digit_u2<C, W>(uw, n, idx, win) : 0;
        const int e = d < 0 ? -d : d;
        uint32_t x2[N], y2[N];
        load_affine<C>(x2, y2, kt + ((size_t)(live ? win : 0) * KT::ENT + (e ? e - 1 : 0)) * EU4);
        pt_add<C, true>(acc, x2, y2, one, d < 0, d == 0);
    }
#pragma unroll 1
    for (int it = 0; it < (C::GWINS + 31) / 32; it++) {
        const int win = it * 32 + (int)lane;
        const bool live = win < C::GWINS;
        const uint32_t b = live ? comb_digit_u1<C>(uw, n, idx, win) : 0u;
        uint32_t x2[N], y2[N];
        load_affine<C>(x2, y2, gtab + (((size_t)(live ? win : 0) << C::GW) + b) * EU4);
        pt_add<C, true>(acc, x2, y2, one, false, b == 0);
    }
#pragma unroll 1
    for (int off = 16; off >= 1; off >>= 1) {
        uint32_t x2[N], y2[N], z2[N];
#pragma unroll
        for (int i = 0; i < N; i++) {
            x2[i] = __shfl_down_sync(0xffffffffu, acc.X[i], off);
            y2[i] = __shfl_down_sync(0xffffffffu, acc.Y[i], off);
            z2[i] = __shfl_down_sync(0xffffffffu, acc.Z[i], off);
        }
        pt_add<C, false>(acc, x2, y2, z2, false, mp_is_zero<N>(z2));
    }
    if (lane != 0) return;
    ok_out[idx] = (good && final_check<C>(acc, r_be, idx)) ? 1 : 0;
}

}
```

consensus_b200/csrc/keygroup.cuh:

```cuda
#pragma once
#include "kernels.cuh"

namespace sbv {

constexpr uint32_t KG_EMPTY = 0xffffffffu;

template <class C>
SBV_DEV uint32_t kg_hash(const uint8_t *__restrict__ qx_be, const uint8_t *__restrict__ qy_be, uint32_t i, uint32_t seed) {
    const uint32_t *x = reinterpret_cast<const uint32_t *>(qx_be + (size_t)i * C::BYTES);
    const uint32_t *y = reinterpret_cast<const uint32_t *>(qy_be + (size_t)i * C::BYTES);
    uint32_t h = seed;
#pragma unroll
    for (int k = 0; k < C::N; k += 2) {
        h = (h ^ __ldg(x + k)) * 0x9E3779B1u;
        h = (h ^ __ldg(y + k + 1)) * 0x85EBCA77u;
        h ^= h >> 15;
    }
    return h;
}
template <class C>
SBV_DEV bool kg_same_key(const uint8_t *__restrict__ qx_be, const uint8_t *__restrict__ qy_be, uint32_t i, uint32_t j) {
    const uint32_t *xi = reinterpret_cast<const uint32_t *>(qx_be + (size_t)i * C::BYTES);
    const uint32_t *xj = reinterpret_cast<const uint32_t *>(qx_be + (size_t)j * C::BYTES);
    const uint32_t *yi = reinterpret_cast<const uint32_t *>(qy_be + (size_t)i * C::BYTES);
    const uint32_t *yj = reinterpret_cast<const uint32_t *>(qy_be + (size_t)j * C::BYTES);
    uint32_t diff = 0;
#pragma unroll
    for (int k = 0; k < C::N; k++) diff |= (__ldg(xi + k) ^ __ldg(xj + k)) | (__ldg(yi + k) ^ __ldg(yj + k));
    return diff == 0;
}

template <class C>
__global__ void __launch_bounds__(256) k_kg_insert(uint32_t n, const uint8_t *__restrict__ qx_be, const uint8_t *__restrict__ qy_be,
                                                   uint32_t seed, uint32_t hmask, uint32_t *__restrict__ htab,
                                                   uint32_t *__restrict__ rep, uint32_t *__restrict__ kcnt) {
    const uint32_t i = blockIdx.x * blockDim.x + threadIdx.x;
    if (i >= n) return;
    uint32_t h = kg_hash<C>(qx_be, qy_be, i, seed) & hmask;
    uint32_t r;
    for (;;) {
        uint32_t cur = htab[h];
        if (cur == KG_EMPTY) {
            cur = atomicCAS(htab + h, KG_EMPTY, i);
            if (cur == KG_EMPTY) { r = i; break; }
        }
        if (kg_same_key<C>(qx_be, qy_be, i, cur)) { r = cur; break; }
        h = (h + 1) & hmask;
    }
    rep[i] = r;
#if defined(__CUDA_ARCH__)
    const uint32_t peers = __match_any_sync(__activemask(), r);
    if ((threadIdx.x & 31) == (uint32_t)(__ffs((int)peers) - 1)) atomicAdd(kcnt + r, (uint32_t)__popc(peers));
#else
    atomicAdd(kcnt + r, 1u);
#endif
}

static __global__ void __launch_bounds__(256) k_kg_assign(uint32_t n, const uint32_t *__restrict__ rep, const uint32_t *__restrict__ kcnt,
                                                   uint32_t threshold, uint32_t max_keys, int32_t *__restrict__ keyid,
                                                   uint32_t *__restrict__ keylist, uint32_t *__restrict__ counters) {
    const uint32_t i = blockIdx.x * blockDim.x + threadIdx.x;
    if (i >= n) return;
    int32_t id = -1;
    if (rep[i] == i && kcnt[i] >= threshold) {
        const uint32_t k = atomicAdd(counters + 0, 1u);
        if (k < max_keys) { id = (int32_t)k; keylist[k] = i; }
    }
    keyid[i] = id;
}

static __global__ void __launch_bounds__(256) k_kg_route(uint32_t n, const uint32_t *__restrict__ rep, const int32_t *__restrict__ keyid,
                                                  int32_t *__restrict__ item_kid, uint32_t *__restrict__ klist, uint32_t *__restrict__ glist,
                                                  uint32_t *__restrict__ counters) {
    const uint32_t i = blockIdx.x * blockDim.x + threadIdx.x;
    const bool live = i < n;
    const int32_t kid = live ? keyid[rep[i]] : -1;
    if (live) item_kid[i] = kid;
#if defined(__CUDA_ARCH__)
    const uint32_t lane = threadIdx.x & 31;
    const uint32_t mk = __ballot_sync(0xffffffffu, live && kid >= 0), mg = __ballot_sync(0xffffffffu, live && kid < 0);
    uint32_t bk = 0, bg = 0;
    if (lane == 0) {
        if (mk) bk = atomicAdd(counters + 1, (uint32_t)__popc(mk));
        if (mg) bg = atomicAdd(counters + 2, (uint32_t)__popc(mg));
    }
    bk = __shfl_sync(0xffffffffu, bk, 0);
    bg = __shfl_sync(0xffffffffu, bg, 0);
    const uint32_t below = (1u << lane) - 1u;
    if (live && kid >= 0) klist[bk + __popc(mk & below)] = i;
    if (live && kid < 0) glist[bg + __popc(mg & below)] = i;
#else
    if (live && kid >= 0) klist[atomicAdd(counters + 1, 1u)] = i;
    if (live && kid < 0) glist[atomicAdd(counters + 2, 1u)] = i;
#endif
}


template <class C, class KT, bool INL>
__global__ void __launch_bounds__(64) k_kt_bases(const uint32_t *__restrict__ nkeys_ptr, uint32_t cap, const uint32_t *__restrict__ keylist,
                                                 const uint8_t *__restrict__ qx_be, const uint8_t *__restrict__ qy_be,
                                                 uint32_t *__restrict__ bases, uint8_t *__restrict__ keyflags) {
    constexpr int N = C::N;
    const uint32_t k = blockIdx.x * blockDim.x + threadIdx.x;
    uint32_t nkeys = __ldg(nkeys_ptr);
    if (nkeys > cap) nkeys = cap;
    if (k >= nkeys) return;
    const uint32_t item = keylist ? keylist[k] : k;
    using A = typename PickArith<C, INL>::type;
    Jac<A> B;
    const bool good = load_key<C>(B.X, B.Y, qx_be, qy_be, item);
    keyflags[k] = good ? 1 : 0;
    if (!good) return;
    C::get_one(B.Z);
#pragma unroll 1
    for (int win = 0; win < KT::NBASE; win++) {
        if (win) {
#pragma unroll 1
            for (int d = 0; d < KT::STEP; d++) pt_double<A>(B);
        }
        uint32_t *o = bases + (size_t)win * 3 * N * cap + k;
#pragma unroll
        for (int i = 0; i < N; i++) { o[(size_t)i * cap] = B.X[i]; o[(size_t)(N + i) * cap] = B.Y[i]; o[(size_t)(2 * N + i) * cap] = B.Z[i]; }
    }
}

template <class C, class KT>
__global__ void __launch_bounds__(128) k_kt_bases4(const uint32_t *__restrict__ nkeys_ptr, uint32_t cap, const uint32_t *__restrict__ keylist,
                                                   const uint8_t *__restrict__ qx_be, const uint8_t *__restrict__ qy_be,
                                                   uint32_t *__restrict__ bases, uint8_t *__restrict__ keyflags) {
    constexpr int N = C::N;
    const uint32_t gt = blockIdx.x * blockDim.x + threadIdx.x;
    const uint32_t k = gt >> 2, role = gt & 3;
    uint32_t nkeys = __ldg(nkeys_ptr);
    if (nkeys > cap) nkeys = cap;
    if (k >= nkeys) return;
    const unsigned qbase = (threadIdx.x & 31) & ~3u, qmask = 0xFu << qbase;
    const uint32_t item = keylist ? keylist[k] : k;
    uint32_t X[N], Y[N], Z[N];
    const bool good = load_key<C>(X, Y, qx_be, qy_be, item);
    if (role == 0) keyflags[k] = good ? 1 : 0;
    if (!good) return;
    C::get_one(Z);
    auto bcast = [&](uint32_t (&v)[N], unsigned src) {
#pragma unroll
        for (int i = 0; i < N; i++) v[i] = __shfl_sync(qmask, v[i], qbase + src);
    };
#pragma unroll 1
    for (int win = 0; win < KT::NBASE; win++) {
        if (win) {
#pragma unroll 1
            for (int d = 0; d < KT::STEP; d++) {
                uint32_t s[N], a[N], b[N], r1[N], r2[N], r3[N], r4[N], t1[N], t2[N];
                C::fadd(s, Y, Y);
                mp_select<N>(a, role == 1 || role == 2, s, Z);
                mp_select<N>(b, role == 1, s, Z);
                C::fmul(r1, a, b);
                uint32_t bb[N];
                mp_copy<N>(bb, r1);
                bcast(bb, 1);
                C::fsub(t1, X, r1);
                C::fadd(t2, X, r1);
                mp_select<N>(a, role == 0, t1, X);
                mp_select<N>(a, role == 2, bb, a);
                mp_select<N>(b, role == 0, t2, bb);
                C::fmul(r2, a, b);
                uint32_t alpha[N], half[N], beta4[N];
                C::fadd(t1, r2, r2);
                C::fadd(alpha, t1, r2);
                C::fhalf(half, r2);
                C::fmul(r3, alpha, alpha);
                mp_copy<N>(beta4, r2);
                bcast(beta4, 1);
                bcast(half, 2);
                uint32_t x3[N], y3[N];
                C::fadd(t1, beta4, beta4);
                C::fsub(x3, r3, t1);
                C::fsub(t2, beta4, x3);
                C::fmul(r4, alpha, t2);
                C::fsub(y3, r4, half);
                mp_copy<N>(X, x3); bcast(X, 0);
                mp_copy<N>(Y, y3); bcast(Y, 0);
                mp_copy<N>(Z, r1); bcast(Z, 2);
            }
        }
        if (role == 0) {
            uint32_t *o = bases + (size_t)win * 3 * N * cap + k;
#pragma unroll
            for (int i = 0; i < N; i++) { o[(size_t)i * cap] = X[i]; o[(size_t)(N + i) * cap] = Y[i]; o[(size_t)(2 * N + i) * cap] = Z[i]; }
        }
    }
}

template <class C>
SBV_DEV void zaddu(uint32_t (&X1)[C::N], uint32_t (&Y1)[C::N], const uint32_t (&X2)[C::N], const uint32_t (&Y2)[C::N],
                   uint32_t (&X3)[C::N], uint32_t (&Y3)[C::N], uint32_t (&h)[C::N]) {
    constexpr int N = C::N;
    uint32_t c[N], w1[N], w2[N], dy[N], d[N], a1[N], t[N];
    C::fsub(h, X1, X2);
    C::fsqr(c, h);
    C::fmul(w1, X1, c);
    C::fmul(w2, X2, c);
    C::fsub(dy, Y1, Y2);
    C::fsqr(d, dy);
    C::fsub(t, w1, w2);
    C::fmul(a1, Y1, t);
    C::fsub(X3, d, w1);
    C::fsub(X3, X3, w2);
    C::fsub(t, w1, X3);
    C::fmul(Y3, dy, t);
    C::fsub(Y3, Y3, a1);
    mp_copy<N>(X1, w1);
    mp_copy<N>(Y1, a1);
}

template <class C, int W>
__global__ void __launch_bounds__(64) k_kt_fill(const uint32_t *__restrict__ nkeys_ptr, uint32_t cap, const uint32_t *__restrict__ bases,
                                                const uint8_t *__restrict__ keyflags, uint32_t *__restrict__ hs,
                                                uint32_t *__restrict__ ztop, uint32_t *__restrict__ ktab) {
    constexpr int N = C::N;
    using KT = KeyTab<32 * N, W>;
    const uint32_t t = blockIdx.x * blockDim.x + threadIdx.x;
    uint32_t nkeys = __ldg(nkeys_ptr);
    if (nkeys > cap) nkeys = cap;
    if (t >= nkeys * KT::NWIN) return;
    const uint32_t k = t % nkeys, win = t / nkeys;
    if (!keyflags[k]) return;
    uint32_t bx[N], by[N], bz[N];
    {
        const uint32_t *o = bases + (size_t)win * 3 * N * cap + k;
#pragma unroll
        for (int i = 0; i < N; i++) { bx[i] = o[(size_t)i * cap]; by[i] = o[(size_t)(N + i) * cap]; bz[i] = o[(size_t)(2 * N + i) * cap]; }
    }
    uint32_t *out = ktab + ((size_t)k * KT::NWIN + win) * KT::ENT * 2 * N;
#pragma unroll
    for (int i = 0; i < N; i++) { out[i] = bx[i]; out[N + i] = by[i]; }
    Jac<C> P;
    mp_copy<N>(P.X, bx); mp_copy<N>(P.Y, by); mp_copy<N>(P.Z, bz);
    uint32_t h[N], h2[N], h3[N];
    C::fadd(h, by, by);
    pt_double<C>(P);
    C::fsqr(h2, h);
    C::fmul(h3, h2, h);
    C::fmul(bx, bx, h2);
    C::fmul(by, by, h3);
    uint32_t zacc[N];
    mp_copy<N>(zacc, P.Z);
    {
        uint32_t *hp = hs + ((size_t)win * (KT::ENT - 1) + 0) * N * cap + k;
#pragma unroll
        for (int i = 0; i < N; i++) { out[2 * N + i] = P.X[i]; out[3 * N + i] = P.Y[i]; hp[(size_t)i * cap] = h[i]; }
    }
    uint32_t px[N], py[N];
    mp_copy<N>(px, P.X); mp_copy<N>(py, P.Y);
#pragma unroll 1
    for (int e = 3; e <= KT::ENT; e++) {
        uint32_t x3[N], y3[N];
        zaddu<C>(bx, by, px, py, x3, y3, h);
        C::fmul(zacc, zacc, h);
        mp_copy<N>(px, x3); mp_copy<N>(py, y3);
        uint32_t *hp = hs + ((size_t)win * (KT::ENT - 1) + (e - 2)) * N * cap + k;
        uint32_t *oe = out + (size_t)(e - 1) * 2 * N;
#pragma unroll
        for (int i = 0; i < N; i++) { oe[i] = px[i]; oe[N + i] = py[i]; hp[(size_t)i * cap] = h[i]; }
    }
    uint32_t *zp = ztop + (size_t)win * N * cap + k;
#pragma unroll
    for (int i = 0; i < N; i++) zp[(size_t)i * cap] = zacc[i];
}

template <class C, class KT>
__global__ void __launch_bounds__(64) k_kt_inv(const uint32_t *__restrict__ nkeys_ptr, uint32_t cap, const uint8_t *__restrict__ keyflags,
                                               uint32_t *__restrict__ ztop, uint32_t *__restrict__ pref) {
    constexpr int N = C::N;
    const uint32_t k = blockIdx.x * blockDim.x + threadIdx.x;
    uint32_t nkeys = __ldg(nkeys_ptr);
    if (nkeys > cap) nkeys = cap;
    if (k >= nkeys || !keyflags[k]) return;
    uint32_t run[N];
    C::get_one(run);
#pragma unroll 1
    for (int win = 0; win < KT::NCHAIN; win++) {
        uint32_t z[N];
        const uint32_t *zp = ztop + (size_t)win * N * cap + k;
        uint32_t *pp = pref + (size_t)win * N * cap + k;
#pragma unroll
        for (int i = 0; i < N; i++) { z[i] = zp[(size_t)i * cap]; pp[(size_t)i * cap] = run[i]; }
        C::fmul(run, run, z);
    }
    uint32_t inv[N];
    p_inv<C>(inv, run);
#pragma unroll 1
    for (int win = KT::NCHAIN - 1; win >= 0; win--) {
        uint32_t z[N], pv[N], zi[N];
        uint32_t *zp = ztop + (size_t)win * N * cap + k;
        const uint32_t *pp = pref + (size_t)win * N * cap + k;
#pragma unroll
        for (int i = 0; i < N; i++) { z[i] = zp[(size_t)i * cap]; pv[i] = pp[(size_t)i * cap]; }
        C::fmul(zi, inv, pv);
        C::fmul(inv, inv, z);
#pragma unroll
        for (int i = 0; i < N; i++) zp[(size_t)i * cap] = zi[i];
    }
}

template <class C, class KT>
__global__ void __launch_bounds__(64) k_kt_final(const uint32_t *__restrict__ nkeys_ptr, uint32_t cap, const uint32_t *__restrict__ bases,
                                                 const uint8_t *__restrict__ keyflags, const uint32_t *__restrict__ hs,
                                                 const uint32_t *__restrict__ ztop, uint32_t *__restrict__ ktab) {
    constexpr int N = C::N;
    const uint32_t t = blockIdx.x * blockDim.x + threadIdx.x;
    uint32_t nkeys = __ldg(nkeys_ptr);
    if (nkeys > cap) nkeys = cap;
    if (t >= nkeys * KT::NCHAIN) return;
    const uint32_t k = t % nkeys, win = t / nkeys;
    if (!keyflags[k]) return;
    uint32_t zi[N];
    {
        const uint32_t *zp = ztop + (size_t)win * N * cap + k;
#pragma unroll
        for (int i = 0; i < N; i++) zi[i] = zp[(size_t)i * cap];
    }
    uint32_t *out = ktab + ((size_t)k * KT::NCHAIN + win) * KT::ENT * 2 * N;
    uint32_t x[N], y[N], h[N];
    {
        const uint32_t *oe = out + (size_t)(KT::ENT - 1) * 2 * N;
#pragma unroll
        for (int i = 0; i < N; i++) { x[i] = oe[i]; y[i] = oe[N + i]; }
    }
#pragma unroll 1
    for (int e = KT::ENT; e >= 1; e--) {
        uint32_t nx[N], ny[N], nh[N];
        if (e >= 2) {
            const uint32_t *on = out + (size_t)(e - 2) * 2 * N;
            const uint32_t *hp = hs + ((size_t)win * (KT::ENT - 1) + (e - 2)) * N * cap + k;
#pragma unroll
            for (int i = 0; i < N; i++) { nx[i] = on[i]; ny[i] = on[N + i]; nh[i] = hp[(size_t)i * cap]; }
        }
        uint32_t *oe = out + (size_t)(e - 1) * 2 * N;
        uint32_t z2[N], z3[N];
        C::fsqr(z2, zi);
        C::fmul(z3, z2, zi);
        C::fmul(x, x, z2);
        C::fmul(y, y, z3);
#pragma unroll
        for (int i = 0; i < N; i++) { oe[i] = x[i]; oe[N + i] = y[i]; }
        if (e >= 2) {
            mp_copy<N>(h, nh);
            C::fmul(zi, zi, h);
            mp_copy<N>(x, nx); mp_copy<N>(y, ny);
        }
    }
    (void)bases;
}


template <class C>
__global__ void __launch_bounds__(64) k_comb_affine(const uint32_t *__restrict__ nkeys_ptr, uint32_t cap, const uint8_t *__restrict__ keyflags,
                                                    uint32_t *__restrict__ bases, uint32_t *__restrict__ pref) {
    constexpr int N = C::N;
    using CT = CombTab<C>;
    const uint32_t k = blockIdx.x * blockDim.x + threadIdx.x;
    uint32_t nkeys = __ldg(nkeys_ptr);
    if (nkeys > cap) nkeys = cap;
    if (k >= nkeys || !keyflags[k]) return;
    uint32_t run[N];
    C::get_one(run);
#pragma unroll 1
    for (int c = 0; c < CT::NBASE; c++) {
        uint32_t z[N];
        const uint32_t *zp = bases + ((size_t)c * 3 + 2) * N * cap + k;
        uint32_t *pp = pref + (size_t)c * N * cap + k;
#pragma unroll
        for (int i = 0; i < N; i++) { z[i] = zp[(size_t)i * cap]; pp[(size_t)i * cap] = run[i]; }
        C::fmul(run, run, z);
    }
    uint32_t inv[N];
    p_inv<C>(inv, run);
#pragma unroll 1
    for (int c = CT::NBASE - 1; c >= 0; c--) {
        uint32_t *o = bases + (size_t)c * 3 * N * cap + k;
        const uint32_t *pp = pref + (size_t)c * N * cap + k;
        uint32_t x[N], y[N], z[N], pv[N], zi[N], z2[N], z3[N];
#pragma unroll
        for (int i = 0; i < N; i++) { x[i] = o[(size_t)i * cap]; y[i] = o[(size_t)(N + i) * cap]; z[i] = o[(size_t)(2 * N + i) * cap]; pv[i] = pp[(size_t)i * cap]; }
        C::fmul(zi, inv, pv);
        C::fmul(inv, inv, z);
        C::fsqr(z2, zi);
        C::fmul(z3, z2, zi);
        C::fmul(x, x, z2);
        C::fmul(y, y, z3);
#pragma unroll
        for (int i = 0; i < N; i++) { o[(size_t)i * cap] = x[i]; o[(size_t)(N + i) * cap] = y[i]; }
    }
}

template <class C>
__global__ void __launch_bounds__(64) k_comb_fill(const uint32_t *__restrict__ nkeys_ptr, uint32_t cap, const uint32_t *__restrict__ bases,
                                                  const uint8_t *__restrict__ keyflags, uint32_t *__restrict__ hs,
                                                  uint32_t *__restrict__ ztop, uint32_t *__restrict__ ktab) {
    constexpr int N = C::N;
    using CT = CombTab<C>;
    const uint32_t t = blockIdx.x * blockDim.x + threadIdx.x;
    uint32_t nkeys = __ldg(nkeys_ptr);
    if (nkeys > cap) nkeys = cap;
    if (t >= nkeys * CT::NCHAIN) return;
    const uint32_t k = t % nkeys, ch = t / nkeys;
    if (!keyflags[k]) return;
    const int b = (int)(ch >> 4), hi = (int)(ch & 15);
    auto base = [&](int c, uint32_t (&x)[N], uint32_t (&y)[N]) {
        const uint32_t *o = bases + (size_t)c * 3 * N * cap + k;
#pragma unroll
        for (int i = 0; i < N; i++) { x[i] = o[(size_t)i * cap]; y[i] = o[(size_t)(N + i) * cap]; }
    };
    uint32_t *out = ktab + ((size_t)k * CT::NCHAIN + ch) * CT::ENT * 2 * N;
    auto store = [&](int slot, const uint32_t (&x)[N], const uint32_t (&y)[N], const uint32_t (&h)[N]) {
        uint32_t *o = out + (size_t)slot * 2 * N;
#pragma unroll
        for (int i = 0; i < N; i++) { o[i] = x[i]; o[N + i] = y[i]; }
        if (slot) {
            uint32_t *hp = hs + ((size_t)ch * (CT::ENT - 1) + (slot - 1)) * N * cap + k;
#pragma unroll
            for (int i = 0; i < N; i++) hp[(size_t)i * cap] = h[i];
        }
    };
    Jac<C> P;
    uint32_t x[N], y[N], h[N];
    C::get_one(P.Z);
    C::get_one(h);
    int first;
    if (hi == 0) {
        uint32_t zero[N];
#pragma unroll
        for (int i = 0; i < N; i++) zero[i] = 0;
        store(0, zero, zero, h);
        base(CT::TEETH * b, P.X, P.Y);
        store(1, P.X, P.Y, h);
        first = 2;
    } else {
        bool empty = true;
#pragma unroll 1
        for (int i = 0; i < 4; i++) {
            if (!((hi >> i) & 1)) continue;
            base(CT::TEETH * b + 4 + i, x, y);
            if (empty) { mp_copy<N>(P.X, x); mp_copy<N>(P.Y, y); empty = false; }
            else pt_madd_table<C>(P, x, y, h);
        }
        store(0, P.X, P.Y, h);
        first = 1;
    }
#pragma unroll 1
    for (int kk = first; kk < CT::ENT; kk++) {
        const int tooth = __ffs(kk) - 1;
        base(CT::TEETH * b + tooth, x, y);
        if (!(((kk ^ (kk >> 1)) >> tooth) & 1)) {
            uint32_t zero[N];
#pragma unroll
            for (int i = 0; i < N; i++) zero[i] = 0;
            C::fsub(y, zero, y);
        }
        pt_madd_table<C>(P, x, y, h);
        store(kk, P.X, P.Y, h);
    }
    uint32_t *zp = ztop + (size_t)ch * N * cap + k;
#pragma unroll
    for (int i = 0; i < N; i++) zp[(size_t)i * cap] = P.Z[i];
}

template <class C, class KT_>
struct KtSizes {
    using KT = KT_;
    static constexpr size_t bases_words(size_t cap) { return (size_t)KT::NBASE * 3 * C::N * cap; }
    static constexpr size_t hs_words(size_t cap) { return (size_t)KT::NCHAIN * (KT::ENT - 1) * C::N * cap; }
    static constexpr size_t ztop_words(size_t cap) { return (size_t)KT::NCHAIN * C::N * cap; }
    static constexpr size_t ktab_words(size_t cap) { return KT::POINTS * 2 * C::N * cap; }
};

}
```

consensus_b200/csrc/ops.h:

```cpp
#pragma once
#include <cuda_runtime.h>
#include <stddef.h>
#include <stdint.h>

struct KtGeom {
    size_t bases_words, hs_words, ztop_words, ktab_words;
};

struct KtOps {
    KtGeom geom;
    cudaError_t (*build)(const uint32_t *nkeys_ptr, uint32_t cap, const uint32_t *keylist, const uint8_t *qx, const uint8_t *qy,
                         uint32_t *bases, uint32_t *hs, uint32_t *ztop, uint32_t *pref, uint32_t *ktab, uint8_t *keyflags, cudaStream_t st);
    cudaError_t (*verify)(int reg, int warp, uint32_t n, const uint32_t *slot, const int32_t *kidmap, uint32_t n_slots,
                          const uint8_t *keyflags, const uint8_t *r, const uint32_t *uw, const uint8_t *flags, const uint32_t *gtab,
                          const uint32_t *ktab, uint8_t *ok, const uint32_t *list, const uint32_t *count, const uint32_t *gacc, cudaStream_t st);
};

struct CurveOps {
    int N, bytes;
    size_t gtab_entries;
    cudaError_t (*gtable_init)(uint32_t *gtab, cudaStream_t st);
    cudaError_t (*prep)(uint32_t n, const uint8_t *r, const uint8_t *s, const uint8_t *dig, uint32_t dlen, uint32_t *uw, uint8_t *flags,
                        cudaStream_t st);
    cudaError_t (*group)(uint32_t n, const uint8_t *qx, const uint8_t *qy, uint32_t seed, uint32_t hmask, uint32_t *htab, uint32_t *rep,
                         uint32_t *kcnt, uint32_t threshold, uint32_t max_keys, int32_t *keyid, uint32_t *keylist, int32_t *item_kid,
                         uint32_t *klist, uint32_t *glist, uint32_t *counters, int route, cudaStream_t st);
    cudaError_t (*route)(uint32_t n, const uint32_t *rep, const int32_t *keyid, int32_t *item_kid, uint32_t *klist, uint32_t *glist,
                         uint32_t *counters, cudaStream_t st);
    cudaError_t (*gpart)(uint32_t n, const uint32_t *uw, const uint32_t *gtab, uint32_t *gacc, cudaStream_t st);
    cudaError_t (*coz)(uint32_t n, const uint8_t *qx, const uint8_t *qy, const uint8_t *r, const uint32_t *uw, const uint8_t *flags,
                       const uint32_t *gtab, uint32_t *tscr, uint8_t *ok, const uint32_t *list, const uint32_t *count, cudaStream_t st);
    const KtOps *grouped, *kt8;
};

#define SBV_COZ_DECL(NAME)                                                                                                          \
    cudaError_t NAME(uint32_t n, const uint8_t *qx, const uint8_t *qy, const uint8_t *r, const uint32_t *uw, const uint8_t *flags, \
                     const uint32_t *gtab, uint32_t *tscr, uint8_t *ok, const uint32_t *list, const uint32_t *count, cudaStream_t st)
SBV_COZ_DECL(sbv_coz_p256);
SBV_COZ_DECL(sbv_coz_p384);
extern const CurveOps sbv_ops_p256, sbv_ops_p384;
extern const KtOps sbv_comb_p256, sbv_kt8_p256, sbv_kt5_p384, sbv_kt8_p384;
inline const CurveOps &sbv_ops(int curve) { return curve == 0 ? sbv_ops_p256 : sbv_ops_p384; }
```

consensus_b200/csrc/pipeline.cu:

```cuda
#include "engine.h"

namespace {

int take_scratch(sbv_engine *e, Dev &d, const CurveOps &ops, const KtOps *kt, size_t n, size_t kcap, cudaStream_t st, Dev::Scratch **out) {
    int idx = (int)(d.ws_next++ % SBV_SCRATCH);
    for (int tries = 0; tries < SBV_SCRATCH && d.ws[idx].open; tries++) idx = (int)(d.ws_next++ % SBV_SCRATCH);
    if (d.ws[idx].open) return sbv_fail(e, SBV_ERR_ARG, "no free scratch set (more launches held open than lanes?)");
    Dev::Scratch &w = d.ws[idx];
    Dev::Scratch::Caps &c = w.caps;
    if (!w.done) {
        for (int j = 0; j < SBV_SCRATCH; j++) {
            Dev::Scratch &x = d.ws[j];
            if (x.done) continue;
            CU(e, cudaEventCreateWithFlags(&x.done, cudaEventDisableTiming));
            CU(e, cudaEventCreateWithFlags(&x.ev_group, cudaEventDisableTiming));
            CU(e, cudaEventCreateWithFlags(&x.ev_prep, cudaEventDisableTiming));
            CU(e, cudaEventCreateWithFlags(&x.ev_tab, cudaEventDisableTiming));
            CU(e, cudaEventCreateWithFlags(&x.ev_gen, cudaEventDisableTiming));
            if (e->tab_hi) {
                int lo_p = 0, hi_p = 0;
                CU(e, cudaDeviceGetStreamPriorityRange(&lo_p, &hi_p));
                CU(e, cudaStreamCreateWithPriority(&x.s_tab, cudaStreamNonBlocking, hi_p));
            } else {
                CU(e, cudaStreamCreateWithFlags(&x.s_tab, cudaStreamNonBlocking));
            }
            CU(e, cudaStreamCreateWithFlags(&x.s_gen, cudaStreamNonBlocking));
        }
    }
    const size_t N = (size_t)ops.N;
    uint32_t hsize = 1;
    while (hsize < 2 * n) hsize <<= 1;
    struct Need { void **p; size_t *cap; size_t need, alloc; };
    const size_t ni = n + n / 8 + 1024, kc = kcap + kcap / 8 + 16;
    uint32_t hs2 = 1;
    while (hs2 < 2 * ni) hs2 <<= 1;
    const bool g = kcap > 0, t = g && kt;
    const KtGeom z{};
    const KtGeom &q = t ? kt->geom : z;
    Need needs[] = {
        {(void **)&w.uw, &c.uw, 2 * N * n * 4, 2 * N * ni * 4},
        {(void **)&w.flags, &c.flags, n, ni},
        {(void **)&w.tscr, &c.tscr, 12 * N * n * 4, 12 * N * ni * 4},
        {(void **)&w.gacc, &c.gacc, g ? 3 * N * n * 4 : 0, 3 * N * ni * 4},
        {(void **)&w.htab, &c.htab, g ? (size_t)hsize * 4 : 0, (size_t)hs2 * 4},
        {(void **)&w.rep, &c.rep, g ? n * 4 : 0, ni * 4},
        {(void **)&w.klist, &c.klist, g ? n * 4 : 0, ni * 4},
        {(void **)&w.glist, &c.glist, g ? n * 4 : 0, ni * 4},
        {(void **)&w.zeroed, &c.zeroed, g ? (n + 4 + 4 * SBV_MAX_CHUNKS) * 4 : 0, (ni + 4 + 4 * SBV_MAX_CHUNKS) * 4},
        {(void **)&w.keyid, &c.keyid, g ? n * 4 : 0, ni * 4},
        {(void **)&w.item_kid, &c.item_kid, g ? n * 4 : 0, ni * 4},
        {(void **)&w.keylist, &c.keylist, t ? kcap * 4 : 0, kc * 4},
        {(void **)&w.keyflags, &c.keyflags, t ? kcap : 0, kc},
        {(void **)&w.bases, &c.bases, q.bases_words * kcap * 4, q.bases_words * kc * 4},
        {(void **)&w.hs, &c.hs, q.hs_words * kcap * 4, q.hs_words * kc * 4},
        {(void **)&w.ztop, &c.ztop, q.ztop_words * kcap * 4, q.ztop_words * kc * 4},
        {(void **)&w.pref, &c.pref, q.ztop_words * kcap * 4, q.ztop_words * kc * 4},
        {(void **)&w.ktab, &c.ktab, q.ktab_words * kcap * 4, q.ktab_words * kc * 4},
    };
    bool grows = false;
    for (const Need &nd : needs) grows = grows || nd.need > *nd.cap;
    if (grows) {
        for (int j = 0; j < SBV_SCRATCH; j++) {
            Dev::Scratch &x = d.ws[j];
            if (x.open && &x != &w) continue;
            if (x.used && x.done) CU(e, cudaEventSynchronize(x.done));
            Dev::Scratch::Caps &cx = x.caps;
            struct Slot { void **p; size_t *cap; };
            const Slot slots[] = {
                {(void **)&x.uw, &cx.uw}, {(void **)&x.flags, &cx.flags}, {(void **)&x.tscr, &cx.tscr}, {(void **)&x.gacc, &cx.gacc},
                {(void **)&x.htab, &cx.htab}, {(void **)&x.rep, &cx.rep}, {(void **)&x.klist, &cx.klist}, {(void **)&x.glist, &cx.glist},
                {(void **)&x.zeroed, &cx.zeroed}, {(void **)&x.keyid, &cx.keyid}, {(void **)&x.item_kid, &cx.item_kid}, {(void **)&x.keylist, &cx.keylist},
                {(void **)&x.keyflags, &cx.keyflags}, {(void **)&x.bases, &cx.bases}, {(void **)&x.hs, &cx.hs}, {(void **)&x.ztop, &cx.ztop},
                {(void **)&x.pref, &cx.pref}, {(void **)&x.ktab, &cx.ktab},
            };
            static_assert(sizeof(slots) / sizeof(slots[0]) == sizeof(needs) / sizeof(needs[0]), "one slot per buffer");
            for (size_t q = 0; q < sizeof(slots) / sizeof(slots[0]); q++) {
                if (needs[q].need <= *slots[q].cap) continue;
                if (*slots[q].p) cudaFree(*slots[q].p);
                *slots[q].p = nullptr;
                *slots[q].cap = 0;
                CU(e, cudaMalloc(slots[q].p, needs[q].alloc));
                *slots[q].cap = needs[q].alloc;
            }
        }
    }
    w.hsize = hsize;
    if (w.used) CU(e, cudaStreamWaitEvent(st, w.done, 0));
    w.used = true;
    *out = &w;
    return 0;
}

cudaEvent_t *prof_take(sbv_engine *e, Dev &d) {
    if (!e->profiling) return nullptr;
    if (d.prof_used + 5 > d.prof_events.size()) {
        size_t old = d.prof_events.size();
        d.prof_events.resize(old + 128);
        for (size_t i = old; i < d.prof_events.size(); i++)
            if (cudaEventCreate(&d.prof_events[i]) != cudaSuccess) { d.prof_events.resize(i); return nullptr; }
    }
    cudaEvent_t *ev = &d.prof_events[d.prof_used];
    d.prof_used += 5;
    return ev;
}

}

void sbv_scratch_free(Dev &d) {
    for (auto &w : d.ws) {
        void *ptrs[] = {w.uw, w.flags, w.tscr, w.gacc, w.htab, w.rep, w.keylist, w.klist, w.glist, w.zeroed, w.keyid, w.item_kid, w.bases, w.hs, w.ztop, w.pref, w.ktab, w.keyflags};
        for (void *p : ptrs) if (p) cudaFree(p);
        cudaEvent_t evs[] = {w.done, w.ev_group, w.ev_prep, w.ev_tab, w.ev_gen};
        for (cudaEvent_t ev : evs) if (ev) cudaEventDestroy(ev);
        if (w.s_tab) cudaStreamDestroy(w.s_tab);
        if (w.s_gen) cudaStreamDestroy(w.s_gen);
        w = Dev::Scratch{};
    }
}

int sbv_init_gtables(sbv_engine *e, Dev &d) {
    for (int c = 0; c < 2; c++) {
        const CurveOps &ops = sbv_ops(c);
        CU(e, cudaMalloc(&d.gtab[c], ops.gtab_entries * 2 * ops.N * 4));
        CU(e, ops.gtable_init(d.gtab[c], d.stream));
    }
    e->launches += 2;
    CU(e, cudaStreamSynchronize(d.stream));
    return 0;
}

int sbv_launch_verify_begin(sbv_engine *e, Dev &d, uint8_t curve, size_t n, const uint8_t *d_qx, const uint8_t *d_qy, cudaStream_t st,
                            VerifyLaunch *vl, int chunks) {
    *vl = VerifyLaunch{};
    if (n == 0) return 0;
    if (chunks < 1 || chunks > SBV_MAX_CHUNKS) return sbv_fail(e, SBV_ERR_ARG, "bad chunk count %d", chunks);
    const CurveOps &ops = sbv_ops(curve);
    const KtOps *kt = ops.grouped;
    const uint32_t nn = (uint32_t)n;
    const uint32_t T = e->group_threshold > 0 ? (uint32_t)e->group_threshold : 0;
    const bool grouping = T > 0 && n >= T && n >= (size_t)e->group_min_batch && e->group_max_keys > 0;
    size_t kcap = 0;
    if (grouping) {
        kcap = n / T;
        if (kcap > (size_t)e->group_max_keys) kcap = (size_t)e->group_max_keys;
        if (kcap == 0) kcap = 1;
    }
    Dev::Scratch *w = nullptr;
    if (int rc = take_scratch(e, d, ops, grouping ? kt : nullptr, n, kcap, st, &w)) return rc;
    w->open = true;
    vl->w = w; vl->curve = curve; vl->n = n; vl->grouping = grouping; vl->d_qx = d_qx; vl->d_qy = d_qy; vl->chunks = chunks;
    vl->ev = prof_take(e, d);
    if (vl->ev) CU(e, cudaEventRecord(vl->ev[0], st));
    if (!grouping) return 0;
    uint32_t *counters = w->zeroed, *kcnt = w->zeroed + 4;
    CU(e, cudaMemsetAsync(w->htab, 0xff, (size_t)w->hsize * 4, st));
    CU(e, cudaMemsetAsync(w->zeroed, 0, (n + 4 + (chunks > 1 ? 4 * chunks : 0)) * 4, st));
    CU(e, ops.group(nn, d_qx, d_qy, e->hash_seed, w->hsize - 1, w->htab, w->rep, kcnt, T, (uint32_t)kcap, w->keyid, w->keylist, w->item_kid, w->klist,
                    w->glist, counters, chunks == 1, st));
    CU(e, cudaEventRecord(w->ev_group, st));
    CU(e, cudaStreamWaitEvent(w->s_tab, w->ev_group, 0));
    CU(e, kt->build(counters + 0, (uint32_t)kcap, w->keylist, d_qx, d_qy, w->bases, w->hs, w->ztop, w->pref, w->ktab, w->keyflags, w->s_tab));
    CU(e, cudaEventRecord(w->ev_tab, w->s_tab));
    e->launches += (chunks == 1 ? 3 : 2) + (curve == 0 ? 5 : 4);
    return 0;
}

int sbv_launch_verify_chunk(sbv_engine *e, Dev &d, const VerifyLaunch &vl, int c, size_t lo, size_t cn, bool last, const uint8_t *d_r, const uint8_t *d_s,
                            const uint8_t *d_dig, uint32_t dlen, uint8_t *d_ok, cudaStream_t st) {
    if (vl.n == 0) return 0;
    Dev::Scratch *w = vl.w;
    if (vl.chunks <= 1 || c < 0 || c >= vl.chunks || lo + cn > vl.n) return sbv_fail(e, SBV_ERR_ARG, "bad chunk");
    const CurveOps &ops = sbv_ops(vl.curve);
    const KtOps *kt = ops.grouped;
    const size_t N = (size_t)ops.N, L = (size_t)ops.bytes;
    const uint32_t nn = (uint32_t)cn;
    const uint32_t *gtab = d.gtab[vl.curve];
    cudaEvent_t *ev = last ? vl.ev : nullptr;
    if (ev) CU(e, cudaEventRecord(ev[0], st));
    uint32_t *uw = w->uw + 2 * N * lo, *tscr = w->tscr + 12 * N * lo;
    uint8_t *flags = w->flags + lo;
    const uint8_t *r = d_r + lo * L;
    if (cn) {
        CU(e, ops.prep(nn, r, d_s + lo * L, d_dig + lo * dlen, dlen, uw, flags, st));
        e->launches += 1;
    }
    if (ev) CU(e, cudaEventRecord(ev[1], st));
    if (!vl.grouping) {
        if (ev) { CU(e, cudaEventRecord(ev[4], st)); CU(e, cudaEventRecord(ev[2], st)); }
        if (cn) {
            CU(e, ops.coz(nn, vl.d_qx + lo * L, vl.d_qy + lo * L, r, uw, flags, gtab, tscr, d_ok + lo, nullptr, nullptr, st));
            e->launches += 1;
        }
        if (ev) CU(e, cudaEventRecord(ev[3], st));
    } else if (cn) {
        uint32_t *cc = w->zeroed + 4 + vl.n + 4 * (size_t)c;
        uint32_t *klist = w->klist + lo, *glist = w->glist + lo;
        CU(e, ops.route(nn, w->rep + lo, w->keyid, w->item_kid + lo, klist, glist, cc, st));
        CU(e, cudaEventRecord(w->ev_prep, st));
        CU(e, cudaStreamWaitEvent(w->s_gen, w->ev_prep, 0));
        CU(e, ops.coz(nn, vl.d_qx + lo * L, vl.d_qy + lo * L, r, uw, flags, gtab, tscr, d_ok + lo, glist, cc + 2, w->s_gen));
        CU(e, cudaEventRecord(w->ev_gen, w->s_gen));
        const uint32_t *gacc = nullptr;
        if (e->gsplit) {
            uint32_t *ga = w->gacc + 3 * N * lo;
            CU(e, ops.gpart(nn, uw, gtab, ga, st));
            gacc = ga;
            e->launches += 1;
        }
        if (ev) CU(e, cudaEventRecord(ev[4], st));
        if (c == 0) CU(e, cudaStreamWaitEvent(st, w->ev_tab, 0));
        if (ev) CU(e, cudaEventRecord(ev[2], st));
        CU(e, kt->verify(0, 0, nn, nullptr, w->item_kid + lo, 0, w->keyflags, r, uw, flags, gtab, w->ktab, d_ok + lo, klist, cc + 1, gacc, st));
        if (ev) CU(e, cudaEventRecord(ev[3], st));
        CU(e, cudaStreamWaitEvent(st, w->ev_gen, 0));
        e->launches += 3;
    } else if (ev) {
        CU(e, cudaEventRecord(ev[4], st)); CU(e, cudaEventRecord(ev[2], st)); CU(e, cudaEventRecord(ev[3], st));
    }
    if (last) {
        CU(e, cudaEventRecord(w->done, st));
        w->open = false;
    }
    return 0;
}

void sbv_launch_verify_abort(const VerifyLaunch &vl, cudaStream_t st) {
    Dev::Scratch *w = vl.w;
    if (!w || !w->open) return;
    if (vl.grouping) cudaStreamWaitEvent(st, w->ev_tab, 0);
    cudaStreamWaitEvent(st, w->ev_gen, 0);
    cudaEventRecord(w->done, st);
    w->open = false;
}

int sbv_launch_verify_finish(sbv_engine *e, Dev &d, const VerifyLaunch &vl, const uint8_t *d_r, const uint8_t *d_s, const uint8_t *d_dig,
                             uint32_t dlen, uint8_t *d_ok, cudaStream_t st) {
    if (vl.n == 0) return 0;
    if (vl.chunks != 1) return sbv_fail(e, SBV_ERR_ARG, "chunked launch finished in one piece");
    const CurveOps &ops = sbv_ops(vl.curve);
    const KtOps *kt = ops.grouped;
    Dev::Scratch *w = vl.w;
    cudaEvent_t *ev = vl.ev;
    const uint32_t nn = (uint32_t)vl.n;
    const uint32_t *gtab = d.gtab[vl.curve];
    CU(e, ops.prep(nn, d_r, d_s, d_dig, dlen, w->uw, w->flags, st));
    if (!vl.grouping) {
        if (ev) { CU(e, cudaEventRecord(ev[1], st)); CU(e, cudaEventRecord(ev[4], st)); CU(e, cudaEventRecord(ev[2], st)); }
        CU(e, ops.coz(nn, vl.d_qx, vl.d_qy, d_r, w->uw, w->flags, gtab, w->tscr, d_ok, nullptr, nullptr, st));
        if (ev) CU(e, cudaEventRecord(ev[3], st));
        CU(e, cudaEventRecord(w->done, st));
        w->open = false;
        e->launches += 2;
        return 0;
    }
    uint32_t *counters = w->zeroed;
    CU(e, cudaEventRecord(w->ev_prep, st));
    if (ev) CU(e, cudaEventRecord(ev[1], st));
    CU(e, cudaStreamWaitEvent(w->s_gen, w->ev_prep, 0));
    CU(e, ops.coz(nn, vl.d_qx, vl.d_qy, d_r, w->uw, w->flags, gtab, w->tscr, d_ok, w->glist, counters + 2, w->s_gen));
    CU(e, cudaEventRecord(w->ev_gen, w->s_gen));
    const uint32_t *gacc = nullptr;
    if (e->gsplit) {
        CU(e, ops.gpart(nn, w->uw, gtab, w->gacc, st));
        gacc = w->gacc;
        e->launches += 1;
    }
    if (ev) CU(e, cudaEventRecord(ev[4], st));
    CU(e, cudaStreamWaitEvent(st, w->ev_tab, 0));
    if (ev) CU(e, cudaEventRecord(ev[2], st));
    CU(e, kt->verify(0, 0, nn, nullptr, w->item_kid, 0, w->keyflags, d_r, w->uw, w->flags, gtab, w->ktab, d_ok, w->klist, counters + 1, gacc, st));
    if (ev) CU(e, cudaEventRecord(ev[3], st));
    CU(e, cudaStreamWaitEvent(st, w->ev_gen, 0));
    CU(e, cudaEventRecord(w->done, st));
    w->open = false;
    e->launches += 3;
    return 0;
}

int sbv_launch_verify(sbv_engine *e, Dev &d, uint8_t curve, size_t n, const uint8_t *d_r, const uint8_t *d_s, const uint8_t *d_qx,
                      const uint8_t *d_qy, const uint8_t *d_dig, uint32_t dlen, uint8_t *d_ok, cudaStream_t st) {
    VerifyLaunch vl;
    if (int rc = sbv_launch_verify_begin(e, d, curve, n, d_qx, d_qy, st, &vl)) return rc;
    return sbv_launch_verify_finish(e, d, vl, d_r, d_s, d_dig, dlen, d_ok, st);
}

void sbv_keys_free(Dev &d) {
    for (int c = 0; c < 2; c++) {
        if (d.ktab[c]) cudaFree(d.ktab[c]);
        if (d.keyflags[c]) cudaFree(d.keyflags[c]);
        if (d.slot2local[c]) cudaFree(d.slot2local[c]);
        d.ktab[c] = nullptr; d.keyflags[c] = nullptr; d.slot2local[c] = nullptr; d.n_local[c] = 0;
    }
    d.n_slots = 0;
}

int sbv_keys_build(sbv_engine *e, Dev &d) {
    CU(e, cudaSetDevice(d.ordinal));
    CU(e, cudaDeviceSynchronize());
    sbv_keys_free(d);
    const size_t n = e->key_ids.size();
    d.n_slots = (uint32_t)n;
    if (n == 0) return 0;
    for (int c = 0; c < 2; c++) {
        const CurveOps &ops = sbv_ops(c);
        const KtOps *kt = ops.kt8;
        const size_t L = (size_t)ops.bytes;
        std::vector<int32_t> map(n, -1);
        std::vector<uint8_t> kx, ky;
        uint32_t cnt = 0;
        for (size_t i = 0; i < n; i++) {
            if (e->key_curve[i] != c) continue;
            const uint8_t *x = &e->key_xy[96 * i], *y = x + 48;
            bool fits = true;
            for (size_t b = 0; b < 48 - L; b++) if (x[b] || y[b]) fits = false;
            if (!fits) continue;
            map[i] = (int32_t)cnt++;
            kx.insert(kx.end(), x + (48 - L), x + 48);
            ky.insert(ky.end(), y + (48 - L), y + 48);
        }
        CU(e, cudaMalloc(&d.slot2local[c], n * sizeof(int32_t)));
        CU(e, cudaMemcpyAsync(d.slot2local[c], map.data(), n * sizeof(int32_t), cudaMemcpyHostToDevice, d.stream));
        d.n_local[c] = cnt;
        if (cnt == 0) { CU(e, cudaStreamSynchronize(d.stream)); continue; }
        CU(e, cudaMalloc(&d.ktab[c], kt->geom.ktab_words * cnt * 4));
        CU(e, cudaMalloc(&d.keyflags[c], cnt));
        uint8_t *d_kx = nullptr, *d_ky = nullptr;
        uint32_t *tmp = nullptr, *d_cnt = nullptr;
        const size_t tmp_words = (kt->geom.bases_words + kt->geom.hs_words + 2 * kt->geom.ztop_words) * cnt;
        CU(e, cudaMalloc(&d_kx, kx.size()));
        CU(e, cudaMalloc(&d_ky, ky.size()));
        CU(e, cudaMalloc(&tmp, tmp_words * 4));
        CU(e, cudaMalloc(&d_cnt, 4));
        CU(e, cudaMemcpyAsync(d_kx, kx.data(), kx.size(), cudaMemcpyHostToDevice, d.stream));
        CU(e, cudaMemcpyAsync(d_ky, ky.data(), ky.size(), cudaMemcpyHostToDevice, d.stream));
        CU(e, cudaMemcpyAsync(d_cnt, &cnt, 4, cudaMemcpyHostToDevice, d.stream));
        uint32_t *bases = tmp, *hs = bases + kt->geom.bases_words * cnt, *ztop = hs + kt->geom.hs_words * cnt, *pref = ztop + kt->geom.ztop_words * cnt;
        cudaError_t st = kt->build(d_cnt, cnt, nullptr, d_kx, d_ky, bases, hs, ztop, pref, d.ktab[c], d.keyflags[c], d.stream);
        e->launches += 4;
        if (st == cudaSuccess) st = cudaStreamSynchronize(d.stream);
        cudaFree(d_kx); cudaFree(d_ky); cudaFree(tmp); cudaFree(d_cnt);
        CU(e, st);
    }
    return 0;
}

int sbv_launch_keyed(sbv_engine *e, Dev &d, uint8_t curve, size_t n, const uint32_t *d_slot, const uint8_t *d_r, const uint8_t *d_s,
                     const uint8_t *d_dig, uint32_t dlen, uint8_t *d_ok, cudaStream_t st) {
    if (n == 0) return 0;
    if (d.n_local[curve] == 0) {
        CU(e, cudaMemsetAsync(d_ok, 0, n, st));
        return 0;
    }
    const CurveOps &ops = sbv_ops(curve);
    const KtOps *kt = ops.kt8;
    const uint32_t nn = (uint32_t)n;
    Dev::Scratch *w = nullptr;
    if (int rc = take_scratch(e, d, ops, nullptr, n, 0, st, &w)) return rc;
    cudaEvent_t *ev = prof_take(e, d);
    if (ev) CU(e, cudaEventRecord(ev[0], st));
    CU(e, ops.prep(nn, d_r, d_s, d_dig, dlen, w->uw, w->flags, st));
    if (ev) { CU(e, cudaEventRecord(ev[1], st)); CU(e, cudaEventRecord(ev[4], st)); CU(e, cudaEventRecord(ev[2], st)); }
    const int warp = nn <= (uint32_t)e->keyed_warp_limit ? 1 : 0;
    CU(e, kt->verify(1, warp, nn, d_slot, d.slot2local[curve], d.n_slots, d.keyflags[curve], d_r, w->uw, w->flags, d.gtab[curve], d.ktab[curve], d_ok,
                     nullptr, nullptr, nullptr, st));
    if (ev) CU(e, cudaEventRecord(ev[3], st));
    CU(e, cudaEventRecord(w->done, st));
    e->launches += 2;
    return 0;
}
```

Before: 67.35 million.

## Use signed-digit comb tables for P-256 per-key grouped verification

Replaces the unsigned comb table for per-key (grouped) P-256 verification with a signed comb. The scalar u2 is made odd by negating it (with a flag bit) and each comb column is read as a signed digit. This halves the table entries per block and removes the zero-digit skip, so each lookup touches a smaller key table. Negation is folded into the point-add sign across the verify kernels. The cost is extra doubled-base storage, a new fill kernel, and a flag encoding that every consumer must honour.

```diff
diff --git a/consensus_b200/csrc/engine.cu b/consensus_b200/csrc/engine.cu
--- a/consensus_b200/csrc/engine.cu
+++ b/consensus_b200/csrc/engine.cu
@@ -385,6 +385,7 @@
     e->group_max_keys = env_int("SBV_GROUP_MAX_KEYS", 8192);
     e->group_min_batch = env_int("SBV_GROUP_MIN_BATCH", 0);
     e->gsplit = env_int("SBV_GSPLIT", 1) != 0;
+    e->comb_signed = env_int("SBV_COMB_SIGNED", 1) != 0;
     e->chunk_items = env_int("SBV_CHUNK_ITEMS", 262144);
     e->gather_hi = env_int("SBV_GATHER_PRIORITY", 1) != 0;
     e->tab_hi = env_int("SBV_TAB_PRIORITY", 1) != 0;
diff --git a/consensus_b200/csrc/engine.h b/consensus_b200/csrc/engine.h
--- a/consensus_b200/csrc/engine.h
+++ b/consensus_b200/csrc/engine.h
@@ -85,6 +85,7 @@
     int group_min_batch = 0;
     int chunk_items = 262144;
     bool gsplit = true;
+    bool comb_signed = true;
     uint32_t hash_seed = 0x9e3779b9u;
     bool profiling = false;
     void *nccl_lib = nullptr;
diff --git a/consensus_b200/csrc/inst_common.cuh b/consensus_b200/csrc/inst_common.cuh
--- a/consensus_b200/csrc/inst_common.cuh
+++ b/consensus_b200/csrc/inst_common.cuh
@@ -96,28 +96,28 @@
     return cudaGetLastError();
 }
 
-template <class C>
+template <class C, class CT>
 cudaError_t op_comb_build(const uint32_t *nkeys_ptr, uint32_t cap, const uint32_t *keylist, const uint8_t *qx, const uint8_t *qy,
                           uint32_t *bases, uint32_t *hs, uint32_t *ztop, uint32_t *pref, uint32_t *ktab, uint8_t *keyflags, cudaStream_t st) {
-    using CT = CombTab<C>;
     const unsigned kb = (cap + 63) / 64;
     const unsigned cb = (unsigned)(((size_t)cap * CT::NCHAIN + 63) / 64);
     k_kt_bases4<C, CT><<<(unsigned)(((size_t)cap * 4 + 127) / 128), 128, 0, st>>>(nkeys_ptr, cap, keylist, qx, qy, bases, keyflags);
-    k_comb_affine<C><<<kb, 64, 0, st>>>(nkeys_ptr, cap, keyflags, bases, pref);
-    k_comb_fill<C><<<cb, 64, 0, st>>>(nkeys_ptr, cap, bases, keyflags, hs, ztop, ktab);
+    k_comb_affine<C, CT><<<kb, 64, 0, st>>>(nkeys_ptr, cap, keyflags, bases, pref);
+    if constexpr (CT::SIGNED) k_scomb_fill<C><<<cb, 64, 0, st>>>(nkeys_ptr, cap, bases, keyflags, hs, ztop, ktab);
+    else k_comb_fill<C><<<cb, 64, 0, st>>>(nkeys_ptr, cap, bases, keyflags, hs, ztop, ktab);
     k_kt_inv<C, CT><<<kb, 64, 0, st>>>(nkeys_ptr, cap, keyflags, ztop, pref);
     k_kt_final<C, CT><<<cb, 64, 0, st>>>(nkeys_ptr, cap, bases, keyflags, hs, ztop, ktab);
     return cudaGetLastError();
 }
 
-template <class C>
+template <class C, class CT>
 cudaError_t op_comb_verify(int reg, int warp, uint32_t n, const uint32_t *slot, const int32_t *kidmap, uint32_t n_slots,
                            const uint8_t *keyflags, const uint8_t *r, const uint32_t *uw, const uint8_t *flags, const uint32_t *gtab,
                            const uint32_t *ktab, uint8_t *ok, const uint32_t *list, const uint32_t *count, const uint32_t *gacc, cudaStream_t st) {
     constexpr int BLOCK = 64;
     (void)slot; (void)n_slots;
     if (reg || warp || !list || !count) return cudaErrorInvalidValue;
-    k_verify_comb<C, BLOCK, Cfg<C>::COMB_MINB, Cfg<C>::COMB_INL><<<(n + BLOCK - 1) / BLOCK, BLOCK, 0, st>>>(
+    k_verify_comb<C, CT, BLOCK, Cfg<C>::COMB_MINB, Cfg<C>::COMB_INL><<<(n + BLOCK - 1) / BLOCK, BLOCK, 0, st>>>(
         n, kidmap, keyflags, r, uw, flags, reinterpret_cast<const uint4 *>(gtab), reinterpret_cast<const uint4 *>(ktab), ok, list, count, gacc);
     return cudaGetLastError();
 }
@@ -125,7 +125,7 @@
 template <class C, class KT>
 constexpr KtGeom kt_geom() {
     using KS = KtSizes<C, KT>;
-    return KtGeom{KS::bases_words(1), KS::hs_words(1), KS::ztop_words(1), KS::ktab_words(1)};
+    return KtGeom{KS::bases_words(1), KS::hs_words(1), KS::ztop_words(1), KS::pref_words(1), KS::ktab_words(1)};
 }
 
 }
diff --git a/consensus_b200/csrc/inst_p256_comb.cu b/consensus_b200/csrc/inst_p256_comb.cu
--- a/consensus_b200/csrc/inst_p256_comb.cu
+++ b/consensus_b200/csrc/inst_p256_comb.cu
@@ -1,3 +1,3 @@
 #include "inst_common.cuh"
 using namespace sbv;
-const KtOps sbv_comb_p256 = {kt_geom<P256, CombTab<P256>>(), op_comb_build<P256>, op_comb_verify<P256>};
+const KtOps sbv_comb_p256 = {kt_geom<P256, SCombTab<P256>>(), op_comb_build<P256, SCombTab<P256>>, op_comb_verify<P256, SCombTab<P256>>};
diff --git a/consensus_b200/csrc/inst_p256_ucomb.cu b/consensus_b200/csrc/inst_p256_ucomb.cu
--- /dev/null
+++ b/consensus_b200/csrc/inst_p256_ucomb.cu
@@ -0,0 +1,3 @@
+#include "inst_common.cuh"
+using namespace sbv;
+const KtOps sbv_ucomb_p256 = {kt_geom<P256, CombTab<P256>>(), op_comb_build<P256, CombTab<P256>>, op_comb_verify<P256, CombTab<P256>>};
diff --git a/consensus_b200/csrc/kernels.cuh b/consensus_b200/csrc/kernels.cuh
--- a/consensus_b200/csrc/kernels.cuh
+++ b/consensus_b200/csrc/kernels.cuh
@@ -110,6 +110,7 @@
     uint32_t run[N];
     C::get_one_n(run);
     int cnt = 0;
+    uint32_t okm = 0;
 #pragma unroll 1
     for (int k = 0; k < S; k++) {
         uint32_t idx = t + (uint32_t)k * T;
@@ -119,6 +120,7 @@
         load_be<N>(r, r_be + (size_t)idx * C::BYTES);
         bool ok = !mp_is_zero<N>(s) && mp_lt<N>(s, nmod) && !mp_is_zero<N>(r) && mp_lt<N>(r, nmod);
         flags[idx] = ok ? 1 : 0;
+        okm |= (ok ? 1u : 0u) << k;
         uint32_t one[N];
 #pragma unroll
         for (int i = 0; i < N; i++) one[i] = (i == 0);
@@ -154,6 +156,12 @@
         load_be<N>(r, r_be + (size_t)idx * C::BYTES);
         C::nmul(u1, e, w);
         C::nmul(u2, r, w);
+        if (((okm >> k) & 1u) && !(u2[0] & 1u)) {
+            uint32_t nu[N];
+            mp_sub<N>(nu, nmod, u2);
+            mp_copy<N>(u2, nu);
+            flags[idx] = 3;
+        }
 #pragma unroll
         for (int i = 0; i < N; i++) {
             uw[(size_t)i * n + idx] = u1[i];
@@ -262,8 +270,15 @@
     C::get_one(one);
     {
         uint32_t qxm[N], qym[N];
-        const bool good = load_key<C>(qxm, qym, qx_be, qy_be, idx) && flags[idx] != 0;
+        const uint8_t fl = flags[idx];
+        const bool good = load_key<C>(qxm, qym, qx_be, qy_be, idx) && (fl & 1);
         if (!good) { ok_out[idx] = 0; return; }
+        if (fl & 2) {
+            uint32_t zero[N];
+#pragma unroll
+            for (int i = 0; i < N; i++) zero[i] = 0;
+            C::fsub(qym, zero, qym);
+        }
         Jac<C> P;
         mp_copy<N>(P.X, qxm); mp_copy<N>(P.Y, qym); mp_copy<N>(P.Z, one);
         pt_double<C>(P);
@@ -348,32 +363,55 @@
     static constexpr int NWIN = Windows<BITS, W>::COUNT;
     static constexpr int ENT = Windows<BITS, W>::ENTRIES;
     static constexpr int NBASE = NWIN, STEP = W, NCHAIN = NWIN;
+    static constexpr int NSTORE = NBASE;
     static constexpr size_t POINTS = (size_t)NWIN * ENT;
+    SBV_DEV static constexpr int dbl_slot(int) { return -1; }
 };
 
 template <class C>
 struct CombTab {
+    static constexpr bool SIGNED = false;
     static constexpr int TEETH = 8, BLOCKS = 2, NBASE = TEETH * BLOCKS;
     static constexpr int SPACING = 32 * C::N / NBASE;
     static constexpr int STEP = SPACING;
+    static constexpr int NSTORE = NBASE;
     static constexpr int NCHAIN = BLOCKS * 16, ENT = 16;
     static constexpr size_t POINTS = (size_t)NCHAIN * ENT;
     static_assert(SPACING * NBASE == 32 * C::N, "the rows cover the scalar exactly");
+    SBV_DEV static constexpr int dbl_slot(int) { return -1; }
     SBV_DEV static uint32_t slot(int b, uint32_t m) {
         const uint32_t g = m & 15u;
         return ((uint32_t)b * 16u + (m >> 4)) * 16u + (g ^ (g >> 1) ^ (g >> 2) ^ (g >> 3));
     }
 };
-
-template <class C>
+template <class C>
+struct SCombTab {
+    static constexpr bool SIGNED = true;
+    static constexpr int TEETH = 8, BLOCKS = 2, NBASE = TEETH * BLOCKS;
+    static constexpr int SPACING = 32 * C::N / NBASE;
+    static constexpr int STEP = SPACING;
+    static constexpr int NSTORE = NBASE + 4 * BLOCKS;
+    static constexpr int NCHAIN = BLOCKS * 8, ENT = 16;
+    static constexpr size_t POINTS = (size_t)NCHAIN * ENT;
+    static_assert(SPACING * NBASE == 32 * C::N, "the rows cover the scalar exactly");
+    SBV_DEV static constexpr int dbl_slot(int c) { return c % TEETH < 4 ? NBASE + 4 * (c / TEETH) + c % TEETH : -1; }
+    SBV_DEV static uint32_t slot(int b, uint32_t m) {
+        const uint32_t g = m & 15u;
+        return ((uint32_t)b * 8u + (m >> 4)) * 16u + (g ^ (g >> 1) ^ (g >> 2) ^ (g >> 3));
+    }
+};
+
+template <class C, class CT>
 SBV_DEV uint32_t comb_mask_u2(const uint32_t *__restrict__ uw, uint32_t n, uint32_t idx, int b, int j) {
-    using CT = CombTab<C>;
+    constexpr int BITS = 32 * C::N;
     const uint32_t *u2 = uw + (size_t)C::N * n + idx;
     uint32_t m = 0;
 #pragma unroll
     for (int t = 0; t < CT::TEETH; t++) {
-        const int pos = CT::SPACING * (CT::TEETH * b + t) + j;
-        m |= ((__ldg(u2 + (size_t)(pos >> 5) * n) >> (pos & 31)) & 1u) << t;
+        const int pos = CT::SPACING * (CT::TEETH * b + t) + j + (CT::SIGNED ? 1 : 0);
+        const int q = pos < BITS ? pos : BITS - 1;
+        const uint32_t bit = pos < BITS ? (__ldg(u2 + (size_t)(q >> 5) * n) >> (q & 31)) & 1u : 1u;
+        m |= bit << t;
     }
     return m;
 }
@@ -422,7 +460,9 @@
     const uint32_t t = blockIdx.x * BLOCK + threadIdx.x;
     if (t >= (list ? __ldg(count) : n)) return;
     const uint32_t idx = list ? __ldg(list + t) : t;
-    bool good = flags[idx] != 0;
+    const uint8_t fl = flags[idx];
+    const bool u2neg = (fl & 2) != 0;
+    bool good = (fl & 1) != 0;
     int32_t kid;
     if (REG) {
         const uint32_t sl = slot[idx];
@@ -454,7 +494,7 @@
             const int d = booth_digit_u2<C, W>(uw, n, idx, w);
             const int e = d < 0 ? -d : d;
             load_affine<C>(x, y, kt + ((size_t)w * KT::ENT + (e ? e - 1 : 0)) * EU4);
-            neg = d < 0; skip = d == 0;
+            neg = (d < 0) != u2neg; skip = d == 0;
         } else {
             const int g = w - KT::NWIN;
             const uint32_t b = comb_digit_u1<C>(uw, n, idx, g);
@@ -478,7 +518,7 @@
     ok_out[idx] = final_check<C>(fin, r_be, idx) ? 1 : 0;
 }
 
-template <class C, int BLOCK, int MINB, bool INL>
+template <class C, class CT, int BLOCK, int MINB, bool INL>
 __global__ void __launch_bounds__(BLOCK, MINB) k_verify_comb(uint32_t n, const int32_t *__restrict__ kidmap, const uint8_t *__restrict__ keyflags,
                                                               const uint8_t *__restrict__ r_be, const uint32_t *__restrict__ uw,
                                                               const uint8_t *__restrict__ flags, const uint4 *__restrict__ gtab,
@@ -488,15 +528,16 @@
     using A = typename PickArith<C, INL>::type;
     constexpr int N = C::N;
     constexpr int EU4 = 2 * N / 4;
-    using CT = CombTab<C>;
     constexpr int KADD = CT::SPACING * CT::BLOCKS;
     const int TOTAL = gacc ? KADD : KADD + C::GWINS;
     const uint32_t t = blockIdx.x * BLOCK + threadIdx.x;
     if (t >= __ldg(count)) return;
     const uint32_t idx = __ldg(list + t);
     const int32_t kid = kidmap[idx];
-    const bool good = flags[idx] != 0 && kid >= 0 && keyflags[kid < 0 ? 0 : kid] != 0;
+    const uint8_t fl = flags[idx];
+    const bool good = (fl & 1) && kid >= 0 && keyflags[kid < 0 ? 0 : kid] != 0;
     if (!good) { ok_out[idx] = 0; return; }
+    const bool u2neg = (fl & 2) != 0;
     const uint4 *kt = ktab + (size_t)kid * CT::POINTS * EU4;
     uint32_t one[N];
     C::get_one(one);
@@ -505,22 +546,31 @@
     mp_copy<N>(acc.Y, one);
 #pragma unroll
     for (int i = 0; i < N; i++) acc.Z[i] = 0;
-    auto fetch = [&](int s, uint32_t (&x)[N], uint32_t (&y)[N], bool &skip) {
+    auto fetch = [&](int s, uint32_t (&x)[N], uint32_t (&y)[N], bool &neg, bool &skip) {
         if (s < KADD) {
             const int b = s & 1;
-            const uint32_t m = comb_mask_u2<C>(uw, n, idx, b, CT::SPACING - 1 - (s >> 1));
-            load_affine<C>(x, y, kt + (size_t)CT::slot(b, m) * EU4);
-            skip = m == 0;
+            const uint32_t m = comb_mask_u2<C, CT>(uw, n, idx, b, CT::SPACING - 1 - (s >> 1));
+            if constexpr (CT::SIGNED) {
+                const bool top = (m >> 7) & 1u;
+                load_affine<C>(x, y, kt + (size_t)CT::slot(b, (top ? m : ~m) & 127u) * EU4);
+                neg = top == u2neg;
+                skip = false;
+            } else {
+                load_affine<C>(x, y, kt + (size_t)CT::slot(b, m) * EU4);
+                neg = u2neg;
+                skip = m == 0;
+            }
         } else {
             const int g = s - KADD;
             const uint32_t d = comb_digit_u1<C>(uw, n, idx, g);
             load_affine<C>(x, y, gtab + (((size_t)g << C::GW) + d) * EU4);
+            neg = false;
             skip = d == 0;
         }
     };
     uint32_t cx[N], cy[N];
-    bool cskip;
-    fetch(0, cx, cy, cskip);
+    bool cneg, cskip;
+    fetch(0, cx, cy, cneg, cskip);
     int s = 0, dbl = 0;
 #pragma unroll 1
     while (s < TOTAL || dbl) {
@@ -530,12 +580,12 @@
             continue;
         }
         uint32_t nx[N], ny[N];
-        bool nskip = true;
-        if (s + 1 < TOTAL) fetch(s + 1, nx, ny, nskip);
-        dbl = pt_add_m<A, 1, true>(acc, cx, cy, one, one, one, false, cskip) ? 1 : 0;
+        bool nneg = false, nskip = true;
+        if (s + 1 < TOTAL) fetch(s + 1, nx, ny, nneg, nskip);
+        dbl = pt_add_m<A, 1, true>(acc, cx, cy, one, one, one, cneg, cskip) ? 1 : 0;
         s++;
         if (s < KADD && (s & 1) == 0) dbl++;
-        if (s < TOTAL) { mp_copy<N>(cx, nx); mp_copy<N>(cy, ny); cskip = nskip; }
+        if (s < TOTAL) { mp_copy<N>(cx, nx); mp_copy<N>(cy, ny); cneg = nneg; cskip = nskip; }
     }
     Jac<C> fin;
     mp_copy<N>(fin.X, acc.X); mp_copy<N>(fin.Y, acc.Y); mp_copy<N>(fin.Z, acc.Z);
@@ -565,7 +615,9 @@
     const uint32_t idx = (blockIdx.x * blockDim.x + threadIdx.x) >> 5;
     const uint32_t lane = threadIdx.x & 31;
     if (idx >= n) return;
-    bool good = flags[idx] != 0;
+    const uint8_t fl = flags[idx];
+    const bool u2neg = (fl & 2) != 0;
+    bool good = (fl & 1) != 0;
     const uint32_t sl = slot[idx];
     int32_t local = sl < n_slots ? slot2local[sl] : -1;
     good = good && local >= 0;
@@ -587,7 +639,7 @@
         const int e = d < 0 ? -d : d;
         uint32_t x2[N], y2[N];
         load_affine<C>(x2, y2, kt + ((size_t)(live ? win : 0) * KT::ENT + (e ? e - 1 : 0)) * EU4);
-        pt_add<C, true>(acc, x2, y2, one, d < 0, d == 0);
+        pt_add<C, true>(acc, x2, y2, one, (d < 0) != u2neg, d == 0);
     }
 #pragma unroll 1
     for (int it = 0; it < (C::GWINS + 31) / 32; it++) {
diff --git a/consensus_b200/csrc/keygroup.cuh b/consensus_b200/csrc/keygroup.cuh
--- a/consensus_b200/csrc/keygroup.cuh
+++ b/consensus_b200/csrc/keygroup.cuh
@@ -112,15 +112,21 @@
     keyflags[k] = good ? 1 : 0;
     if (!good) return;
     C::get_one(B.Z);
+    auto store = [&](int sl) {
+        uint32_t *o = bases + (size_t)sl * 3 * N * cap + k;
+#pragma unroll
+        for (int i = 0; i < N; i++) { o[(size_t)i * cap] = B.X[i]; o[(size_t)(N + i) * cap] = B.Y[i]; o[(size_t)(2 * N + i) * cap] = B.Z[i]; }
+    };
 #pragma unroll 1
     for (int win = 0; win < KT::NBASE; win++) {
         if (win) {
 #pragma unroll 1
-            for (int d = 0; d < KT::STEP; d++) pt_double<A>(B);
-        }
-        uint32_t *o = bases + (size_t)win * 3 * N * cap + k;
-#pragma unroll
-        for (int i = 0; i < N; i++) { o[(size_t)i * cap] = B.X[i]; o[(size_t)(N + i) * cap] = B.Y[i]; o[(size_t)(2 * N + i) * cap] = B.Z[i]; }
+            for (int d = 0; d < KT::STEP; d++) {
+                pt_double<A>(B);
+                if (d == 0 && KT::dbl_slot(win - 1) >= 0) store(KT::dbl_slot(win - 1));
+            }
+        }
+        store(win);
     }
 }
 
@@ -144,6 +150,11 @@
     auto bcast = [&](uint32_t (&v)[N], unsigned src) {
 #pragma unroll
         for (int i = 0; i < N; i++) v[i] = __shfl_sync(qmask, v[i], qbase + src);
+    };
+    auto store = [&](int sl) {
+        uint32_t *o = bases + (size_t)sl * 3 * N * cap + k;
+#pragma unroll
+        for (int i = 0; i < N; i++) { o[(size_t)i * cap] = X[i]; o[(size_t)(N + i) * cap] = Y[i]; o[(size_t)(2 * N + i) * cap] = Z[i]; }
     };
 #pragma unroll 1
     for (int win = 0; win < KT::NBASE; win++) {
@@ -181,13 +192,10 @@
                 mp_copy<N>(X, x3); bcast(X, 0);
                 mp_copy<N>(Y, y3); bcast(Y, 0);
                 mp_copy<N>(Z, r1); bcast(Z, 2);
+                if (role == 0 && d == 0 && KT::dbl_slot(win - 1) >= 0) store(KT::dbl_slot(win - 1));
             }
         }
-        if (role == 0) {
-            uint32_t *o = bases + (size_t)win * 3 * N * cap + k;
-#pragma unroll
-            for (int i = 0; i < N; i++) { o[(size_t)i * cap] = X[i]; o[(size_t)(N + i) * cap] = Y[i]; o[(size_t)(2 * N + i) * cap] = Z[i]; }
-        }
+        if (role == 0) store(win);
     }
 }
 
@@ -354,11 +362,10 @@
 }
 
 
-template <class C>
+template <class C, class CT>
 __global__ void __launch_bounds__(64) k_comb_affine(const uint32_t *__restrict__ nkeys_ptr, uint32_t cap, const uint8_t *__restrict__ keyflags,
                                                     uint32_t *__restrict__ bases, uint32_t *__restrict__ pref) {
     constexpr int N = C::N;
-    using CT = CombTab<C>;
     const uint32_t k = blockIdx.x * blockDim.x + threadIdx.x;
     uint32_t nkeys = __ldg(nkeys_ptr);
     if (nkeys > cap) nkeys = cap;
@@ -366,7 +373,7 @@
     uint32_t run[N];
     C::get_one(run);
 #pragma unroll 1
-    for (int c = 0; c < CT::NBASE; c++) {
+    for (int c = 0; c < CT::NSTORE; c++) {
         uint32_t z[N];
         const uint32_t *zp = bases + ((size_t)c * 3 + 2) * N * cap + k;
         uint32_t *pp = pref + (size_t)c * N * cap + k;
@@ -377,7 +384,7 @@
     uint32_t inv[N];
     p_inv<C>(inv, run);
 #pragma unroll 1
-    for (int c = CT::NBASE - 1; c >= 0; c--) {
+    for (int c = CT::NSTORE - 1; c >= 0; c--) {
         uint32_t *o = bases + (size_t)c * 3 * N * cap + k;
         const uint32_t *pp = pref + (size_t)c * N * cap + k;
         uint32_t x[N], y[N], z[N], pv[N], zi[N], z2[N], z3[N];
@@ -395,6 +402,63 @@
 }
 
 template <class C>
+__global__ void __launch_bounds__(64) k_scomb_fill(const uint32_t *__restrict__ nkeys_ptr, uint32_t cap, const uint32_t *__restrict__ bases,
+                                                   const uint8_t *__restrict__ keyflags, uint32_t *__restrict__ hs,
+                                                   uint32_t *__restrict__ ztop, uint32_t *__restrict__ ktab) {
+    constexpr int N = C::N;
+    using CT = SCombTab<C>;
+    const uint32_t t = blockIdx.x * blockDim.x + threadIdx.x;
+    uint32_t nkeys = __ldg(nkeys_ptr);
+    if (nkeys > cap) nkeys = cap;
+    if (t >= nkeys * CT::NCHAIN) return;
+    const uint32_t k = t % nkeys, ch = t / nkeys;
+    if (!keyflags[k]) return;
+    const int b = (int)(ch >> 3), hi = (int)(ch & 7);
+    auto base = [&](int sl, bool neg, uint32_t (&x)[N], uint32_t (&y)[N]) {
+        const uint32_t *o = bases + (size_t)sl * 3 * N * cap + k;
+#pragma unroll
+        for (int i = 0; i < N; i++) { x[i] = o[(size_t)i * cap]; y[i] = o[(size_t)(N + i) * cap]; }
+        uint32_t zero[N], ny[N];
+#pragma unroll
+        for (int i = 0; i < N; i++) zero[i] = 0;
+        C::fsub(ny, zero, y);
+        mp_select<N>(y, neg, ny, y);
+    };
+    uint32_t *out = ktab + ((size_t)k * CT::NCHAIN + ch) * CT::ENT * 2 * N;
+    auto store = [&](int slot, const uint32_t (&x)[N], const uint32_t (&y)[N], const uint32_t (&h)[N]) {
+        uint32_t *o = out + (size_t)slot * 2 * N;
+#pragma unroll
+        for (int i = 0; i < N; i++) { o[i] = x[i]; o[N + i] = y[i]; }
+        if (slot) {
+            uint32_t *hp = hs + ((size_t)ch * (CT::ENT - 1) + (slot - 1)) * N * cap + k;
+#pragma unroll
+            for (int i = 0; i < N; i++) hp[(size_t)i * cap] = h[i];
+        }
+    };
+    Jac<C> P;
+    uint32_t x[N], y[N], h[N];
+    base(CT::TEETH * b + 7, false, P.X, P.Y);
+    C::get_one(P.Z);
+#pragma unroll 1
+    for (int i = 0; i < 7; i++) {
+        const int tooth = i < 3 ? 4 + i : i - 3;
+        base(CT::TEETH * b + tooth, i < 3 ? !((hi >> i) & 1) : true, x, y);
+        pt_madd_table<C>(P, x, y, h);
+    }
+    store(0, P.X, P.Y, h);
+#pragma unroll 1
+    for (int kk = 1; kk < CT::ENT; kk++) {
+        const int tooth = __ffs(kk) - 1;
+        base(CT::dbl_slot(CT::TEETH * b + tooth), !(((kk ^ (kk >> 1)) >> tooth) & 1), x, y);
+        pt_madd_table<C>(P, x, y, h);
+        store(kk, P.X, P.Y, h);
+    }
+    uint32_t *zp = ztop + (size_t)ch * N * cap + k;
+#pragma unroll
+    for (int i = 0; i < N; i++) zp[(size_t)i * cap] = P.Z[i];
+}
+
+template <class C>
 __global__ void __launch_bounds__(64) k_comb_fill(const uint32_t *__restrict__ nkeys_ptr, uint32_t cap, const uint32_t *__restrict__ bases,
                                                   const uint8_t *__restrict__ keyflags, uint32_t *__restrict__ hs,
                                                   uint32_t *__restrict__ ztop, uint32_t *__restrict__ ktab) {
@@ -469,9 +533,10 @@
 template <class C, class KT_>
 struct KtSizes {
     using KT = KT_;
-    static constexpr size_t bases_words(size_t cap) { return (size_t)KT::NBASE * 3 * C::N * cap; }
+    static constexpr size_t bases_words(size_t cap) { return (size_t)KT::NSTORE * 3 * C::N * cap; }
     static constexpr size_t hs_words(size_t cap) { return (size_t)KT::NCHAIN * (KT::ENT - 1) * C::N * cap; }
     static constexpr size_t ztop_words(size_t cap) { return (size_t)KT::NCHAIN * C::N * cap; }
+    static constexpr size_t pref_words(size_t cap) { return (size_t)(KT::NSTORE > KT::NCHAIN ? KT::NSTORE : KT::NCHAIN) * C::N * cap; }
     static constexpr size_t ktab_words(size_t cap) { return KT::POINTS * 2 * C::N * cap; }
 };
 
diff --git a/consensus_b200/csrc/ops.h b/consensus_b200/csrc/ops.h
--- a/consensus_b200/csrc/ops.h
+++ b/consensus_b200/csrc/ops.h
@@ -4,7 +4,7 @@
 #include <stdint.h>
 
 struct KtGeom {
-    size_t bases_words, hs_words, ztop_words, ktab_words;
+    size_t bases_words, hs_words, ztop_words, pref_words, ktab_words;
 };
 
 struct KtOps {
@@ -39,5 +39,5 @@
 SBV_COZ_DECL(sbv_coz_p256);
 SBV_COZ_DECL(sbv_coz_p384);
 extern const CurveOps sbv_ops_p256, sbv_ops_p384;
-extern const KtOps sbv_comb_p256, sbv_kt8_p256, sbv_kt5_p384, sbv_kt8_p384;
+extern const KtOps sbv_comb_p256, sbv_ucomb_p256, sbv_kt8_p256, sbv_kt5_p384, sbv_kt8_p384;
 inline const CurveOps &sbv_ops(int curve) { return curve == 0 ? sbv_ops_p256 : sbv_ops_p384; }
diff --git a/consensus_b200/csrc/pipeline.cu b/consensus_b200/csrc/pipeline.cu
--- a/consensus_b200/csrc/pipeline.cu
+++ b/consensus_b200/csrc/pipeline.cu
@@ -54,7 +54,7 @@
         {(void **)&w.bases, &c.bases, q.bases_words * kcap * 4, q.bases_words * kc * 4},
         {(void **)&w.hs, &c.hs, q.hs_words * kcap * 4, q.hs_words * kc * 4},
         {(void **)&w.ztop, &c.ztop, q.ztop_words * kcap * 4, q.ztop_words * kc * 4},
-        {(void **)&w.pref, &c.pref, q.ztop_words * kcap * 4, q.ztop_words * kc * 4},
+        {(void **)&w.pref, &c.pref, q.pref_words * kcap * 4, q.pref_words * kc * 4},
         {(void **)&w.ktab, &c.ktab, q.ktab_words * kcap * 4, q.ktab_words * kc * 4},
     };
     bool grows = false;
@@ -91,6 +91,10 @@
     return 0;
 }
 
+const KtOps *grouped_ops(const sbv_engine *e, uint8_t curve) {
+    return curve == 0 && !e->comb_signed ? &sbv_ucomb_p256 : sbv_ops(curve).grouped;
+}
+
 cudaEvent_t *prof_take(sbv_engine *e, Dev &d) {
     if (!e->profiling) return nullptr;
     if (d.prof_used + 5 > d.prof_events.size()) {
@@ -135,7 +139,7 @@
     if (n == 0) return 0;
     if (chunks < 1 || chunks > SBV_MAX_CHUNKS) return sbv_fail(e, SBV_ERR_ARG, "bad chunk count %d", chunks);
     const CurveOps &ops = sbv_ops(curve);
-    const KtOps *kt = ops.grouped;
+    const KtOps *kt = grouped_ops(e, curve);
     const uint32_t nn = (uint32_t)n;
     const uint32_t T = e->group_threshold > 0 ? (uint32_t)e->group_threshold : 0;
     const bool grouping = T > 0 && n >= T && n >= (size_t)e->group_min_batch && e->group_max_keys > 0;
@@ -171,7 +175,7 @@
     Dev::Scratch *w = vl.w;
     if (vl.chunks <= 1 || c < 0 || c >= vl.chunks || lo + cn > vl.n) return sbv_fail(e, SBV_ERR_ARG, "bad chunk");
     const CurveOps &ops = sbv_ops(vl.curve);
-    const KtOps *kt = ops.grouped;
+    const KtOps *kt = grouped_ops(e, vl.curve);
     const size_t N = (size_t)ops.N, L = (size_t)ops.bytes;
     const uint32_t nn = (uint32_t)cn;
     const uint32_t *gtab = d.gtab[vl.curve];
@@ -238,7 +242,7 @@
     if (vl.n == 0) return 0;
     if (vl.chunks != 1) return sbv_fail(e, SBV_ERR_ARG, "chunked launch finished in one piece");
     const CurveOps &ops = sbv_ops(vl.curve);
-    const KtOps *kt = ops.grouped;
+    const KtOps *kt = grouped_ops(e, vl.curve);
     Dev::Scratch *w = vl.w;
     cudaEvent_t *ev = vl.ev;
     const uint32_t nn = (uint32_t)vl.n;
@@ -326,7 +330,7 @@
         CU(e, cudaMalloc(&d.keyflags[c], cnt));
         uint8_t *d_kx = nullptr, *d_ky = nullptr;
         uint32_t *tmp = nullptr, *d_cnt = nullptr;
-        const size_t tmp_words = (kt->geom.bases_words + kt->geom.hs_words + 2 * kt->geom.ztop_words) * cnt;
+        const size_t tmp_words = (kt->geom.bases_words + kt->geom.hs_words + kt->geom.ztop_words + kt->geom.pref_words) * cnt;
         CU(e, cudaMalloc(&d_kx, kx.size()));
         CU(e, cudaMalloc(&d_ky, ky.size()));
         CU(e, cudaMalloc(&tmp, tmp_words * 4));
```

Result: faster. 72.73 million, median of 6 (+8.0%).
